# ljubobratovicrelja/tensor-truth

Hardware: AMD Instinct MI355X
Metric: queries/sec (embed+top-k+rerank) over 10M x 1024 corpus (higher is better)
Workload: dtype bf16

## Files before the change

tensor-truth_amd/csrc/scan.h:

```cpp
#pragma once
#include "common.h"

struct ScanParams {
    const uint16_t* corpus;
    const uint16_t* queries;
    int64_t row_lo, row_hi;
    int n_queries;
    int32_t idx_base;
    float* dense;
    int64_t dense_stride;
    const float* thr;
    int32_t* cnt;
    float* cand_scores;
    int32_t* cand_idx;
    int cap;
    uint2* priv;
    int32_t* priv_cnt;
    int64_t group_stride;
    int64_t phys_rows;
    int prof_id;
    const int32_t* row_table;
    const int32_t* row_cnt;
    const int32_t* gather_rows;
    const int32_t* row_range;
};

#define TT_SCAN_PRIV_SLOTS 16
#define TT_SCAN_WAVES_PER_BLOCK 8
#define TT_SCAN_MAX_SEGMENTS 64
#define TT_SCAN_MAX_PIECES 256

int tt_scan_launch(const ScanParams& p, int dim, int mode, int out, int blocks, hipStream_t stream);

struct SelectParams {
    const float* scores;
    const int32_t* idx;
    int64_t stride;
    const int32_t* cnt;
    int m_fixed;
    int cap;
    int32_t idx_base;
    int k;
    float* out_scores;
    int32_t* out_idx;
    int64_t out_stride;
    const uint2* priv;
    const int32_t* priv_cnt;
    int n_sub;
    float* thr_out;
    int32_t* cnt_out;
    int32_t* overflow_flag;
    int min_valid;
    int thr_relax;
    int32_t* zero_cnt;
    int n_real;
    int n_seg;
    int32_t seg_off[TT_SCAN_MAX_PIECES + 1];
    int32_t seg_add[TT_SCAN_MAX_PIECES];
};

int tt_select_launch(const SelectParams& p, int n_queries, hipStream_t stream);

int tt_lexical_score_lists(const int32_t* q_terms, const float* q_weights, const int32_t* q_start, const int32_t* q_nnz, int n_q,
                           const int32_t* d_terms, const float* d_weights, const int64_t* d_start, const int32_t* d_nnz,
                           const int32_t* cand, const int32_t* cand_cnt, int64_t stride, int grid_cand, float dead, float* out_lex,
                           hipStream_t stream);
bool tt_select_fused_outputs(int k);
```

tensor-truth_amd/csrc/scan.hip:

```cpp
#include "common.h"
#include "scan.h"

namespace {

constexpr int kThreads = 512;
constexpr int kWaves = kThreads / TT_WAVE;
constexpr int kBM = 64;
constexpr int kNG = kBM / 32;
constexpr int kScratchPerWave = 4096;
constexpr int kPrivSlots = TT_SCAN_PRIV_SLOTS;

template <int D>
struct Cfg {
    static constexpr int kRowBytes = D * 2;
    static constexpr int kQImageBytes = kBM * kRowBytes;
    static constexpr int NCH = D / 64;
    static constexpr int NKS = D / 16;
    static constexpr int P1 = (NCH % 4 == 0) ? 4 : ((NCH % 6 == 0) ? 6 : 2);
    static constexpr int P0 = (NKS % 16 == 0) ? 16 : 8;
};

__device__ __forceinline__ uint4 ldg16(const uint16_t* p) {
    return *reinterpret_cast<const uint4*>(p);
}

typedef __attribute__((ext_vector_type(4))) unsigned int u32x4;
template <bool NT>
__device__ __forceinline__ uint4 ldg16c(const uint16_t* p) {
    if constexpr (NT) {
        const u32x4 v = __builtin_nontemporal_load(reinterpret_cast<const u32x4*>(p));
        return make_uint4(v[0], v[1], v[2], v[3]);
    } else {
        return *reinterpret_cast<const uint4*>(p);
    }
}

template <int OUT>
__device__ __forceinline__ void scan_epilogue(const ScanParams& p, f32x16 (&acc)[2], const float (&thr)[2],
                                              const bool (&qvalid)[2], int q0, int ql, int half, int64_t grp,
                                              int (&pcnt)[2], uint2* const (&pbase)[2]) {
    const int64_t row0 = p.row_lo + grp * 32;
    const bool tail = row0 + 32 > p.row_hi;
#pragma unroll
    for (int g = 0; g < 2; ++g) {
        const int q = q0 + g * 32 + ql;
        if constexpr (OUT == 2) {
            float mx = acc[g][0];
#pragma unroll
            for (int r = 1; r < 16; ++r) mx = fmaxf(mx, acc[g][r]);
            mx = fmaxf(mx, __shfl_xor(mx, 32, 64));
            if (qvalid[g] && half == 0) p.dense[(size_t)q * p.dense_stride + (size_t)grp] = mx;
        } else if constexpr (OUT == 1) {
            if (qvalid[g]) {
                float* dst = p.dense + (size_t)q * p.dense_stride + (size_t)(row0 - p.row_lo);
#pragma unroll
                for (int j = 0; j < 4; ++j) {
                    float4 v = make_float4(acc[g][4 * j], acc[g][4 * j + 1], acc[g][4 * j + 2], acc[g][4 * j + 3]);
                    *reinterpret_cast<float4*>(dst + 8 * j + 4 * half) = v;
                }
            }
        } else {
            const float t = thr[g];
            float mx = acc[g][0];
#pragma unroll
            for (int r = 1; r < 16; ++r) mx = fmaxf(mx, acc[g][r]);
            if (__any(mx >= t)) {
#pragma unroll
                for (int r = 0; r < 16; ++r) {
                    const int64_t row = row0 + (r & 3) + 8 * (r >> 2) + 4 * half;
                    bool ok = acc[g][r] >= t;
                    if (tail) ok = ok && (row < p.row_hi);
                    if (ok) {
                        const uint2 e = make_uint2(__float_as_uint(acc[g][r]), (uint32_t)(p.idx_base + (int32_t)row));
                        if (pcnt[g] < kPrivSlots) {
                            pbase[g][pcnt[g]] = e;
                        } else {
                            const int pos = atomicAdd(p.cnt + q, 1);
                            if (pos < p.cap) {
                                p.cand_scores[(size_t)q * p.cap + pos] = acc[g][r];
                                p.cand_idx[(size_t)q * p.cap + pos] = (int32_t)e.y;
                            }
                        }
                        ++pcnt[g];
                    }
                }
            }
        }
#pragma unroll
        for (int r = 0; r < 16; ++r) acc[g][r] = 0.f;
    }
}

template <int D, int MODE, int OUT, int VAR, bool G = false>
__global__ __launch_bounds__(kThreads) void scan_kernel(ScanParams p) {
    using C = Cfg<D>;
    extern __shared__ __attribute__((aligned(16))) char smem[];
    char* q_img = smem;
    const int tid = threadIdx.x;
    const int lane = tid & 63;
    const int wave = __builtin_amdgcn_readfirstlane(tid >> 6);
    char* scratch = smem + C::kQImageBytes + wave * kScratchPerWave;

    const int q0 = blockIdx.y * kBM;

    {
        constexpr int kPiecesPerRow = D / 8;
        constexpr int kPieces = kBM * kPiecesPerRow;
        for (int t = tid; t < kPieces; t += kThreads) {
            const int q = t / kPiecesPerRow;
            const int c = t % kPiecesPerRow;
            uint4 v = make_uint4(0, 0, 0, 0);
            if (q0 + q < p.n_queries) v = ldg16(p.queries + (size_t)(q0 + q) * D + c * 8);
            *reinterpret_cast<uint4*>(q_img + q * C::kRowBytes + ((c ^ (q & 15)) << 4)) = v;
        }
    }
    __syncthreads();

    const int ql = lane & 31;
    const int half = lane >> 5;
    float thr[kNG];
    bool qvalid[kNG];
#pragma unroll
    for (int g = 0; g < kNG; ++g) {
        const int q = q0 + g * 32 + ql;
        qvalid[g] = q < p.n_queries;
        thr[g] = __builtin_inff();
        if (OUT == 0 && qvalid[g]) thr[g] = p.thr[q];
    }
    int qoff[kNG];
#pragma unroll
    for (int g = 0; g < kNG; ++g) qoff[g] = (g * 32 + ql) * C::kRowBytes;
    const int qswz = ql & 15;

    if constexpr (MODE == 0) {
        if (p.row_cnt) {
            const int64_t n = *p.row_cnt;
            p.row_hi = p.row_lo + (n < p.row_hi - p.row_lo ? n : p.row_hi - p.row_lo);
            if (p.row_hi <= p.row_lo) return;
        }
    }
    const int32_t* gtab = nullptr;
    if constexpr (G) {
        const int32_t b = p.row_range[0];
        const int64_t n = (int64_t)p.row_range[1] - b;
        const int64_t span = p.row_hi - p.row_lo;
        p.row_hi = p.row_lo + (n < 0 ? 0 : (n < span ? n : span));
        gtab = p.gather_rows + b;
    }
    const int64_t n_groups = (p.row_hi - p.row_lo + 31) / 32;
    const int64_t per_blk = n_groups / gridDim.x;
    const int64_t rem = n_groups % gridDim.x;
    const int64_t b = blockIdx.x;
    const int64_t g_lo = b * per_blk + (b < rem ? b : rem);
    const int64_t g_hi = g_lo + per_blk + (b < rem ? 1 : 0);

    const uint16_t* corpus = p.corpus;
    const int64_t gstride = (OUT == 2 && p.group_stride > 1) ? p.group_stride : 1;
    const int64_t last_row = (OUT == 2 && p.group_stride > 1) ? p.phys_rows - 1 : p.row_hi - 1;

    f32x16 acc[kNG];
#pragma unroll
    for (int g = 0; g < kNG; ++g)
#pragma unroll
        for (int r = 0; r < 16; ++r) acc[g][r] = 0.f;

    int64_t grp = g_lo + wave;
    const int n_sub = gridDim.x * kWaves * 2;
    const int sub = (blockIdx.x * kWaves + wave) * 2 + half;
    int pcnt[kNG];
    uint2* pbase[kNG];
#pragma unroll
    for (int g = 0; g < kNG; ++g) {
        pcnt[g] = 0;
        pbase[g] = nullptr;
        if (OUT == 0) pbase[g] = p.priv + ((size_t)(q0 + g * 32 + ql) * n_sub + sub) * kPrivSlots;
    }

    if constexpr (MODE == 1) {
        constexpr int P = C::P1;
        uint4 ring[P][4];
        const int lrow = lane >> 3;
        const int lpiece = lane & 7;
        int32_t grow[4] = {0, 0, 0, 0}, grow_n[4] = {0, 0, 0, 0};
        auto gload = [&](int32_t(&dst)[4], int64_t g) {
#pragma unroll
            for (int j = 0; j < 4; ++j) {
                int64_t row = p.row_lo + g * 32 + 8 * j + lrow;
                row = row < last_row ? row : last_row;
                dst[j] = gtab[row];
            }
        };
        auto issue = [&](uint4(&dst)[4], int64_t g, int c, const int32_t(&gr)[4]) {
#pragma unroll
            for (int j = 0; j < 4; ++j) {
                int64_t row;
                if constexpr (G) {
                    row = gr[j];
                } else {
                    row = p.row_lo + g * gstride * 32 + 8 * j + lrow;
                    row = row < last_row ? row : last_row;
                }
                dst[j] = ldg16c<(VAR & 1) == 0>(corpus + (size_t)row * D + c * 64 + lpiece * 8);
            }
        };
        int woff[4];
#pragma unroll
        for (int j = 0; j < 4; ++j) {
            const int row = 8 * j + lrow;
            woff[j] = row * 128 + ((lpiece ^ ((row >> 1) & 7)) << 4);
        }
        const int rbase = ql * 128;
        const int rswz = (ql >> 1) & 7;

        if (grp < g_hi) {
            if constexpr (G) gload(grow, grp);
#pragma unroll
            for (int c = 0; c < P; ++c) issue(ring[c], grp, c, grow);
        }
        while (grp < g_hi) {
            const int64_t nxt = grp + kWaves;
            const bool has_next = nxt < g_hi;
            if constexpr (G) {
                if (has_next) gload(grow_n, nxt);
            }
#pragma unroll
            for (int c = 0; c < C::NCH; ++c) {
                const int s = c % P;
                if constexpr ((VAR & 2) == 0) {
#pragma unroll
                    for (int j = 0; j < 4; ++j)
                        *reinterpret_cast<uint4*>(scratch + woff[j]) = ring[s][j];
                } else {
#pragma unroll
                    for (int j = 0; j < 4; ++j)
                        asm volatile("" ::"v"(ring[s][j].x), "v"(ring[s][j].y), "v"(ring[s][j].z), "v"(ring[s][j].w));
                }
                __builtin_amdgcn_sched_barrier(0);
                if (c + P < C::NCH) {
                    issue(ring[s], grp, c + P, grow);
                } else if (has_next) {
                    issue(ring[s], nxt, c + P - C::NCH, grow_n);
                }
                __builtin_amdgcn_sched_barrier(0);
                if constexpr ((VAR & 6) == 0)
#pragma unroll
                for (int ks = 0; ks < 4; ++ks) {
                    const int piece = 2 * ks + half;
                    const uint4 av = *reinterpret_cast<const uint4*>(scratch + rbase + ((piece ^ rswz) << 4));
                    const bf16x8 a = __builtin_bit_cast(bf16x8, av);
                    const int kc = c * 8 + piece;
#pragma unroll
                    for (int g = 0; g < kNG; ++g) {
                        if constexpr ((VAR & 16) != 0) {
                            acc[g] = __builtin_amdgcn_mfma_f32_32x32x16_bf16(a, a, acc[g], 0, 0, 0);
                        } else {
                            const uint4 bv = *reinterpret_cast<const uint4*>(q_img + qoff[g] + ((kc ^ qswz) << 4));
                            if constexpr ((VAR & 8) != 0) {
                                asm volatile("" ::"v"(bv.x), "v"(bv.y), "v"(bv.z), "v"(bv.w), "v"(av.x), "v"(av.w));
                            } else {
                                acc[g] = __builtin_amdgcn_mfma_f32_32x32x16_bf16(a, __builtin_bit_cast(bf16x8, bv), acc[g], 0, 0, 0);
                            }
                        }
                    }
                }
            }
            scan_epilogue<OUT>(p, acc, thr, qvalid, q0, ql, half, grp, pcnt, pbase);
            grp = nxt;
            if constexpr (G) {
#pragma unroll
                for (int j = 0; j < 4; ++j) grow[j] = grow_n[j];
            }
        }
    } else {
        constexpr int P = C::P0;
        uint4 ring[P];
        auto phys = [&](int64_t g) {
            int64_t row = p.row_lo + g * gstride * 32 + ql;
            const int64_t last = p.row_table ? p.row_hi - 1 : last_row;
            row = row < last ? row : last;
            return p.row_table ? (int64_t)p.row_table[row] : row;
        };
        int64_t row_cur = grp < g_hi ? phys(grp) : 0, row_nxt = 0;
        auto issue = [&](uint4& dst, int64_t row, int ks) {
            dst = ldg16c<(VAR & 1) == 0>(corpus + (size_t)row * D + ks * 16 + half * 8);
        };
        if (grp < g_hi) {
#pragma unroll
            for (int k = 0; k < P; ++k) issue(ring[k], row_cur, k);
        }
        while (grp < g_hi) {
            const int64_t nxt = grp + kWaves;
            const bool has_next = nxt < g_hi;
            if (has_next) row_nxt = phys(nxt);
#pragma unroll
            for (int ks = 0; ks < C::NKS; ++ks) {
                const int s = ks % P;
                const bf16x8 a = __builtin_bit_cast(bf16x8, ring[s]);
                const int kc = 2 * ks + half;
                bf16x8 bfr[kNG];
#pragma unroll
                for (int g = 0; g < kNG; ++g) {
                    const uint4 bv = *reinterpret_cast<const uint4*>(q_img + qoff[g] + ((kc ^ qswz) << 4));
                    bfr[g] = __builtin_bit_cast(bf16x8, bv);
                }
#pragma unroll
                for (int g = 0; g < kNG; ++g)
                    acc[g] = __builtin_amdgcn_mfma_f32_32x32x16_bf16(a, bfr[g], acc[g], 0, 0, 0);
                __builtin_amdgcn_sched_barrier(0);
                if (ks + P < C::NKS) {
                    issue(ring[s], row_cur, ks + P);
                } else if (has_next) {
                    issue(ring[s], row_nxt, ks + P - C::NKS);
                }
                __builtin_amdgcn_sched_barrier(0);
            }
            scan_epilogue<OUT>(p, acc, thr, qvalid, q0, ql, half, grp, pcnt, pbase);
            grp = nxt;
            row_cur = row_nxt;
        }
    }
    if constexpr (OUT == 0) {
#pragma unroll
        for (int g = 0; g < kNG; ++g)
            p.priv_cnt[(size_t)(q0 + g * 32 + ql) * n_sub + sub] = pcnt[g] < kPrivSlots ? pcnt[g] : kPrivSlots;
    }
}

}

template <int D, int MODE, int OUT, int VAR, bool G = false>
static int launch_one(const ScanParams& p, int blocks, int q_tiles, hipStream_t stream) {
    using C = Cfg<D>;
    const size_t lds = (size_t)C::kQImageBytes + (MODE == 1 ? (size_t)kWaves * kScratchPerWave : 0);
    auto kern = scan_kernel<D, MODE, OUT, VAR, G>;
    TT_SET_MAX_LDS(kern, lds);
    {
        TtProfScope prof(p.prof_id ? p.prof_id : (OUT == 0 ? TT_K_SCAN_FILTER : TT_K_SCAN_SAMPLE), stream);
        hipLaunchKernelGGL(kern, dim3(blocks, q_tiles), dim3(kThreads), lds, stream, p);
    }
    TT_CHECK_LAUNCH();
    return TT_OK;
}

template <int D>
static int launch_d(const ScanParams& p, int mode, int out, int blocks, int q_tiles, hipStream_t stream) {
    const int load_mode = mode & 15;
    const int var = mode >> 4;
    if (p.row_range) {
        switch (out) {
            case 0: return launch_one<D, 1, 0, 0, true>(p, blocks, q_tiles, stream);
            case 1: return launch_one<D, 1, 1, 0, true>(p, blocks, q_tiles, stream);
            default: return launch_one<D, 1, 2, 0, true>(p, blocks, q_tiles, stream);
        }
    }
    if constexpr (D == 1024) {
        if (out == 0 && load_mode == 1) {
            switch (var) {
                case 1: return launch_one<D, 1, 0, 1>(p, blocks, q_tiles, stream);
#if TT_DIAG
                case 2: return launch_one<D, 1, 0, 2>(p, blocks, q_tiles, stream);
                case 4: return launch_one<D, 1, 0, 4>(p, blocks, q_tiles, stream);
                case 8: return launch_one<D, 1, 0, 8>(p, blocks, q_tiles, stream);
#endif
                default: break;
            }
        }
    }
    if (load_mode == 1) {
        switch (out) {
            case 0: return launch_one<D, 1, 0, 0>(p, blocks, q_tiles, stream);
            case 1: return launch_one<D, 1, 1, 0>(p, blocks, q_tiles, stream);
            default: return launch_one<D, 1, 2, 0>(p, blocks, q_tiles, stream);
        }
    }
    switch (out) {
        case 0: return launch_one<D, 0, 0, 0>(p, blocks, q_tiles, stream);
        case 1: return launch_one<D, 0, 1, 0>(p, blocks, q_tiles, stream);
        default: return launch_one<D, 0, 2, 0>(p, blocks, q_tiles, stream);
    }
}

int tt_scan_launch(const ScanParams& p, int dim, int mode, int out, int blocks, hipStream_t stream) {
    const int q_tiles = (p.n_queries + kBM - 1) / kBM;
    if (p.row_hi <= p.row_lo || q_tiles == 0) return TT_OK;
    const int64_t n_groups = (p.row_hi - p.row_lo + 31) / 32;
    const int64_t max_blocks = out != 0 ? n_groups : (n_groups + kWaves - 1) / kWaves;
    if (blocks > max_blocks) blocks = (int)max_blocks;
    if (blocks < 1) blocks = 1;
    switch (dim) {
        case 128: return launch_d<128>(p, mode, out, blocks, q_tiles, stream);
        case 256: return launch_d<256>(p, mode, out, blocks, q_tiles, stream);
        case 384: return launch_d<384>(p, mode, out, blocks, q_tiles, stream);
        case 512: return launch_d<512>(p, mode, out, blocks, q_tiles, stream);
        case 640: return launch_d<640>(p, mode, out, blocks, q_tiles, stream);
        case 768: return launch_d<768>(p, mode, out, blocks, q_tiles, stream);
        case 896: return launch_d<896>(p, mode, out, blocks, q_tiles, stream);
        case 1024: return launch_d<1024>(p, mode, out, blocks, q_tiles, stream);
        default:
            tt_set_error("tt_scan: dim %d not in the compiled set {128,256,...,1024: multiples of 128}", dim);
            return TT_E_UNSUPPORTED;
    }
}
```

tensor-truth_amd/csrc/scan_api.hip:

```cpp
#include <limits.h>
#include <string.h>

#include "common.h"
#include "scan.h"
#include "encoder.h"
#include "shadow.h"

static thread_local char g_err[512] = "";

void tt_set_error(const char* fmt, ...) {
    va_list ap;
    va_start(ap, fmt);
    vsnprintf(g_err, sizeof(g_err), fmt, ap);
    va_end(ap);
}

int tt_cu_count_cached() {
    static thread_local int cached_dev = -1;
    static thread_local int cached_cus = 0;
    int dev = 0;
    if (hipGetDevice(&dev) != hipSuccess) return -1;
    if (dev != cached_dev) {
        int cus = 0;
        if (hipDeviceGetAttribute(&cus, hipDeviceAttributeMultiprocessorCount, dev) != hipSuccess) return -1;
        cached_dev = dev;
        cached_cus = cus;
    }
    return cached_cus;
}

namespace {

constexpr int kCap = 16384;
constexpr int64_t kSampleRows = 32768;

struct Plan {
    bool gemm;
    int q256;
    int cap;
    size_t off_q256;
    bool dense_only;
    int64_t n0;
    int64_t stride;
    int qpad;
    int main_blocks;
    int n_sub;
    size_t off_dense, off_cs, off_ci, off_cnt, off_thr, off_priv, off_pcnt, total;
};

int filter_blocks(int64_t rows, int cus) {
    const int64_t groups = (rows + 31) / 32;
    const int64_t mb = (groups + TT_SCAN_WAVES_PER_BLOCK - 1) / TT_SCAN_WAVES_PER_BLOCK;
    int64_t b = cus > 0 ? cus : 256;
    if (b > mb) b = mb;
    if (b < 1) b = 1;
    return (int)b;
}

bool scan_gemm_enabled() {
    static const bool on = TT_DIAG_ENV_INT("TT_SCAN_GEMM", 1) != 0;
    return on;
}

Plan make_plan(int64_t n_rows, int dim, int n_queries, int k, int cus, bool allow_gemm = true) {
    Plan pl{};
    pl.qpad = (n_queries + 63) / 64 * 64;
    pl.cap = kCap;
    int64_t n0 = kSampleRows;
    if (n0 < (int64_t)128 * k) n0 = (int64_t)128 * k;
    pl.gemm = allow_gemm && scan_gemm_enabled() && n_queries > 64 && dim % 128 == 0 && n_rows >= 262144 && n_rows >= (int64_t)2048 * k;
    if (pl.gemm) {
        static const int64_t n0_env = TT_DIAG_ENV_INT("TT_SCAN_GEMM_N0", 0);
        n0 = n0_env > 0 ? n0_env : 131072;
        if (n0_env <= 0)
            while (n0 > 32768 && n0 * 64 > n_rows) n0 /= 2;
        if (n0 < (int64_t)512 * k) n0 = (int64_t)512 * k;
        if (n0 > n_rows / 2) n0 = n_rows / 2 / 32 * 32;
        n0 = n0 / 256 * 256;
        pl.q256 = (n_queries + 255) / 256 * 256;
        pl.qpad = pl.q256;
        int64_t cap = 4 * (int64_t)k * n_rows / n0 + 4096;
        if (cap < kCap) cap = kCap;
        if (cap > (1 << 20)) cap = 1 << 20;
        pl.cap = (int)((cap + 63) / 64 * 64);
    }
    if (n_rows < (int64_t)128 * k || n_rows <= 8192) {
        pl.dense_only = true;
        pl.n0 = n_rows;
        pl.stride = (n_rows + 31) / 32 * 32;
    } else {
        pl.dense_only = false;
        pl.n0 = n0 < n_rows ? n0 : n_rows;
        pl.stride = ((pl.n0 + 31) / 32 + 31) / 32 * 32;
    }
    size_t off = 0;
    pl.off_dense = off; off += tt_align_up((size_t)pl.qpad * pl.stride * sizeof(float), 256);
    pl.off_cs = off;    off += tt_align_up((size_t)pl.qpad * pl.cap * sizeof(float), 256);
    pl.off_ci = off;    off += tt_align_up((size_t)pl.qpad * pl.cap * sizeof(int32_t), 256);
    pl.off_cnt = off;   off += tt_align_up((size_t)pl.qpad * sizeof(int32_t), 256);
    pl.off_thr = off;   off += tt_align_up((size_t)pl.qpad * sizeof(float), 256);
    if (pl.gemm) {
        pl.off_q256 = off; off += tt_align_up((size_t)pl.q256 * dim * sizeof(uint16_t), 256);
        pl.main_blocks = 1;
        pl.n_sub = TT_SCAN_WAVES_PER_BLOCK * 2;
        pl.off_priv = off; off += tt_align_up((size_t)pl.qpad * pl.n_sub * TT_SCAN_PRIV_SLOTS * sizeof(uint2), 256);
        pl.off_pcnt = off; off += tt_align_up((size_t)pl.qpad * pl.n_sub * sizeof(int32_t), 256);
    } else if (!pl.dense_only) {
        pl.main_blocks = filter_blocks(n_rows, cus);
        pl.n_sub = pl.main_blocks * TT_SCAN_WAVES_PER_BLOCK * 2;
        pl.off_priv = off; off += tt_align_up((size_t)pl.qpad * pl.n_sub * TT_SCAN_PRIV_SLOTS * sizeof(uint2), 256);
        pl.off_pcnt = off; off += tt_align_up((size_t)pl.qpad * pl.n_sub * sizeof(int32_t), 256);
    }
    pl.total = off;
    return pl;
}

int check_common(const void* corpus, int64_t n_rows, int dim, const void* queries, int n_queries, int k,
                 const float* out_scores, const int32_t* out_idx) {
    TT_CHECK_ARG(n_rows >= 0 && n_rows < (int64_t)INT32_MAX, "n_rows=%lld out of range", (long long)n_rows);
    TT_CHECK_ARG(n_queries >= 0, "n_queries=%d", n_queries);
    TT_CHECK_ARG(k >= 1 && k <= 1024, "k=%d outside [1,1024]", k);
    TT_CHECK_ARG(dim > 0 && dim % 128 == 0 && dim <= 1024, "dim=%d must be a multiple of 128 and <= 1024", dim);
    if (n_queries == 0) return TT_OK;
    TT_CHECK_ARG(out_scores && out_idx, "null output pointer");
    TT_CHECK_ARG(queries && ((uintptr_t)queries % 16) == 0, "queries must be non-null and 16-byte aligned");
    if (n_rows > 0) TT_CHECK_ARG(corpus && ((uintptr_t)corpus % 16) == 0, "corpus must be non-null and 16-byte aligned");
    return TT_OK;
}

__global__ void relax_thr_kernel(float* thr, int n) {
    const int i = blockIdx.x * blockDim.x + threadIdx.x;
    if (i < n) {
        const float t = thr[i];
        if (t - t == 0.f) thr[i] = t - (fabsf(t) * 1.220703125e-4f + 2e-6f);
    }
}

__global__ void fill_f32_kernel(float* s, float v, int n) {
    const int i = blockIdx.x * blockDim.x + threadIdx.x;
    if (i < n) s[i] = v;
}

__global__ void fill_pad_kernel(float* s, int32_t* ix, int64_t n) {
    const int64_t i = (int64_t)blockIdx.x * blockDim.x + threadIdx.x;
    if (i < n) {
        s[i] = -__builtin_inff();
        ix[i] = -1;
    }
}

int scan_mode_from_env() {
#if TT_DIAG
    const char* e = getenv("TT_SCAN_MODE");
    if (e && e[0]) return atoi(e);
#endif
    return 1;
}

struct ShadowLayout { size_t off_be, off_dn, total; };
ShadowLayout shadow_layout(int64_t cap_rows, int dim) {
    ShadowLayout l{};
    const size_t r16 = (size_t)(cap_rows + 15) / 16 * 16;
    size_t off = tt_align_up((size_t)cap_rows * dim, 256);
    l.off_be = off; off += tt_align_up(r16 * sizeof(float), 256);
    l.off_dn = off; off += tt_align_up(r16 * sizeof(float), 256);
    l.total = off;
    return l;
}
struct ShadowPlan {
    int64_t n0, stride;
    int blocks, n_waves, capw, cap;
    size_t off_sample, off_ss, off_si, off_thr, off_planes, off_qinfo, off_list, off_wcnt, off_table, off_tcnt, off_dense, total;
};
ShadowPlan shadow_plan(int64_t n_rows, int dim, int n_queries, int k, int cus) {
    ShadowPlan pl{};
    int64_t n0 = kSampleRows;
    if (n0 < (int64_t)128 * k) n0 = (int64_t)128 * k;
    if (n0 < n_rows / 32) n0 = n_rows / 32 / 32 * 32;
    pl.n0 = n0 < n_rows ? n0 : n_rows;
    pl.stride = ((pl.n0 + 31) / 32 + 31) / 32 * 32;
    pl.blocks = cus > 0 ? cus : 256;
    const int64_t groups = (n_rows + 15) / 16;
    if ((int64_t)pl.blocks * kShadowWavesPerBlock > groups) pl.blocks = (int)((groups + kShadowWavesPerBlock - 1) / kShadowWavesPerBlock);
    if (pl.blocks < 1) pl.blocks = 1;
    pl.n_waves = pl.blocks * kShadowWavesPerBlock;
    int64_t cap = n_rows / 16;
    if (cap < 65536) cap = 65536;
    if (cap > (1 << 20)) cap = 1 << 20;
    if (cap > (n_rows + 31) / 32 * 32) cap = (n_rows + 31) / 32 * 32;
    pl.cap = (int)((cap + 31) / 32 * 32);
    int64_t capw = 4 * (int64_t)pl.cap / pl.n_waves;
    if (capw < 64) capw = 64;
    pl.capw = (int)capw;
    const int qpad = 64;
    size_t off = 0;
    auto take = [&](size_t bytes) { size_t o = off; off += tt_align_up(bytes, 256); return o; };
    pl.off_sample = take((size_t)qpad * pl.stride * sizeof(float));
    pl.off_ss = take((size_t)qpad * k * sizeof(float));
    pl.off_si = take((size_t)qpad * k * sizeof(int32_t));
    pl.off_thr = take((size_t)qpad * sizeof(float));
    pl.off_planes = take((size_t)(dim / 128) * 4 * 1024);
    pl.off_qinfo = take(32 * sizeof(float));
    pl.off_list = take((size_t)n_queries * pl.n_waves * pl.capw * sizeof(int32_t));
    pl.off_wcnt = take((size_t)n_queries * pl.n_waves * sizeof(int32_t));
    pl.off_table = take((size_t)n_queries * pl.cap * sizeof(int32_t));
    pl.off_tcnt = take((size_t)qpad * sizeof(int32_t));
    pl.off_dense = take((size_t)pl.cap * sizeof(float));
    pl.total = off;
    return pl;
}
__global__ void add_idx_base_kernel(int32_t* idx, int n, int32_t base) {
    const int i = blockIdx.x * blockDim.x + threadIdx.x;
    if (i < n && idx[i] >= 0) idx[i] += base;
}

bool rows_dense(int64_t bound, int k) { return bound < (int64_t)128 * k || bound <= 8192; }
size_t rows_head_bytes(int n_queries) { return tt_align_up((size_t)((n_queries + 63) / 64 * 64) * sizeof(int32_t), 256); }
size_t rows_body_bytes(int64_t bound, int dim, int n_queries, int k, int cus) {
    if (bound <= 0) return 0;
    if (rows_dense(bound, k)) return tt_align_up((size_t)((n_queries + 63) / 64 * 64) * (size_t)((bound + 31) / 32 * 32) * sizeof(float), 256);
    return make_plan(bound, dim, n_queries, k, cus, false).total;
}
__global__ void rows_count_kernel(const int32_t* off, int s, int64_t bound, int32_t* cnt_q, int n, int32_t* flag) {
    const int i = blockIdx.x * blockDim.x + threadIdx.x;
    const int64_t c = (int64_t)off[s + 1] - off[s];
    if (i < n) cnt_q[i] = (int32_t)(c < bound ? c : bound);
    if (i == 0 && c > bound && flag) atomicOr(flag, 8);
}
__global__ void rows_map_kernel(int32_t* idx, int n_queries, int k, int64_t stride, const int32_t* rows, const int32_t* off, int s, int32_t add) {
    const int i = blockIdx.x * blockDim.x + threadIdx.x;
    if (i >= n_queries * k) return;
    int32_t* e = idx + (size_t)(i / k) * stride + (i % k);
    const int32_t pos = *e;
    if (pos >= 0) *e = rows[(int64_t)off[s] + pos] + add;
}
__global__ void fill_pad_strided_kernel(float* s, int32_t* ix, int n_queries, int width, int64_t stride) {
    const int i = blockIdx.x * blockDim.x + threadIdx.x;
    if (i < n_queries * width) {
        const size_t o = (size_t)(i / width) * stride + (i % width);
        s[o] = -__builtin_inff();
        ix[o] = -1;
    }
}
}

extern "C" {

int tt_version(void) { return 1; }
const char* tt_arch(void) { return "gfx950"; }
const char* tt_last_error(void) { return g_err; }
int tt_device_cu_count(void) { return tt_cu_count_cached(); }

size_t tt_scan_workspace_bytes(int64_t n_rows, int dim, int n_queries, int k) {
    if (n_rows < 0 || n_queries <= 0 || k < 1) return 0;
    int cus = tt_cu_count_cached();
    if (cus <= 0) cus = 256;
    return make_plan(n_rows, dim, n_queries, k, cus).total;
}

size_t tt_scan_exact_workspace_bytes(int64_t n_rows, int dim, int n_queries, int k) {
    (void)dim; (void)k;
    if (n_rows < 0 || n_queries <= 0) return 0;
    const int qpad = (n_queries + 63) / 64 * 64;
    const int64_t stride = (n_rows + 31) / 32 * 32;
    return tt_align_up((size_t)qpad * stride * sizeof(float), 256);
}

static int scan_dense_select(const void* corpus, int64_t n_rows, int dim, const void* queries, int n_queries,
                             int k, int32_t idx_base, float* out_scores, int32_t* out_idx, float* dense,
                             int64_t stride, hipStream_t st) {
    ScanParams sp{};
    sp.corpus = (const uint16_t*)corpus;
    sp.queries = (const uint16_t*)queries;
    sp.row_lo = 0;
    sp.row_hi = n_rows;
    sp.n_queries = n_queries;
    sp.idx_base = idx_base;
    sp.dense = dense;
    sp.dense_stride = stride;
    int rc = tt_scan_launch(sp, dim, scan_mode_from_env(), 1, tt_cu_count_cached(), st);
    if (rc) return rc;
    SelectParams se{};
    se.scores = dense;
    se.idx = nullptr;
    se.stride = stride;
    se.cnt = nullptr;
    se.m_fixed = (int)n_rows;
    se.cap = INT_MAX;
    se.idx_base = idx_base;
    se.k = k;
    se.out_scores = out_scores;
    se.out_idx = out_idx;
    se.out_stride = k;
    return tt_select_launch(se, n_queries, st);
}

int tt_scan_topk_exact(const void* corpus_bf16, int64_t n_rows, int dim, const void* queries_bf16,
                       int n_queries, int k, int32_t idx_base, float* out_scores, int32_t* out_idx,
                       void* workspace, size_t workspace_bytes, void* stream) {
    int rc = check_common(corpus_bf16, n_rows, dim, queries_bf16, n_queries, k, out_scores, out_idx);
    if (rc) return rc;
    if (n_queries == 0) return TT_OK;
    hipStream_t st = (hipStream_t)stream;
    if (n_rows == 0) {
        const int64_t n = (int64_t)n_queries * k;
        hipLaunchKernelGGL(fill_pad_kernel, dim3((unsigned)((n + 255) / 256)), dim3(256), 0, st, out_scores, out_idx, n);
        TT_CHECK_LAUNCH();
        return TT_OK;
    }
    const size_t need = tt_scan_exact_workspace_bytes(n_rows, dim, n_queries, k);
    if (!workspace || workspace_bytes < need) {
        tt_set_error("tt_scan_topk_exact: workspace %zu < required %zu bytes", workspace_bytes, need);
        return TT_E_WORKSPACE;
    }
    const int64_t stride = (n_rows + 31) / 32 * 32;
    return scan_dense_select(corpus_bf16, n_rows, dim, queries_bf16, n_queries, k, idx_base, out_scores, out_idx,
                             (float*)workspace, stride, st);
}

int tt_scan_topk(const void* corpus_bf16, int64_t n_rows, int dim, const void* queries_bf16, int n_queries,
                 int k, int32_t idx_base, float* out_scores, int32_t* out_idx, void* workspace,
                 size_t workspace_bytes, int32_t* status_flag, void* stream) {
    int rc = check_common(corpus_bf16, n_rows, dim, queries_bf16, n_queries, k, out_scores, out_idx);
    if (rc) return rc;
    if (n_queries == 0) return TT_OK;
    hipStream_t st = (hipStream_t)stream;
    if (status_flag) TT_CHECK_HIP(hipMemsetAsync(status_flag, 0, sizeof(int32_t), st));
    if (n_rows == 0) {
        const int64_t n = (int64_t)n_queries * k;
        hipLaunchKernelGGL(fill_pad_kernel, dim3((unsigned)((n + 255) / 256)), dim3(256), 0, st, out_scores, out_idx, n);
        TT_CHECK_LAUNCH();
        return TT_OK;
    }
    int cus_plan = tt_cu_count_cached();
    if (cus_plan <= 0) cus_plan = 256;
    const Plan pl = make_plan(n_rows, dim, n_queries, k, cus_plan);
    if (!workspace || workspace_bytes < pl.total) {
        tt_set_error("tt_scan_topk: workspace %zu < required %zu bytes", workspace_bytes, pl.total);
        return TT_E_WORKSPACE;
    }
    TT_CHECK_ARG(((uintptr_t)workspace % 256) == 0, "workspace must be 256-byte aligned");
    char* ws = (char*)workspace;
    float* dense = (float*)(ws + pl.off_dense);
    if (pl.dense_only) {
        return scan_dense_select(corpus_bf16, n_rows, dim, queries_bf16, n_queries, k, idx_base, out_scores,
                                 out_idx, dense, pl.stride, st);
    }
    float* cs = (float*)(ws + pl.off_cs);
    int32_t* ci = (int32_t*)(ws + pl.off_ci);
    int32_t* cnt = (int32_t*)(ws + pl.off_cnt);
    float* thr = (float*)(ws + pl.off_thr);
    const int mode = scan_mode_from_env();
    const int cus = tt_cu_count_cached();

    const uint16_t* q256 = (const uint16_t*)queries_bf16;
    if (pl.gemm && n_queries != pl.q256) {
        uint16_t* qpad256 = (uint16_t*)(ws + pl.off_q256);
        TT_CHECK_HIP(hipMemsetAsync(qpad256 + (size_t)n_queries * dim, 0, (size_t)(pl.q256 - n_queries) * dim * sizeof(uint16_t), st));
        TT_CHECK_HIP(hipMemcpyAsync(qpad256, queries_bf16, (size_t)n_queries * dim * sizeof(uint16_t), hipMemcpyDeviceToDevice, st));
        q256 = qpad256;
    }
    ScanParams sp{};
    sp.corpus = (const uint16_t*)corpus_bf16;
    sp.queries = (const uint16_t*)queries_bf16;
    sp.row_lo = 0;
    sp.row_hi = pl.n0;
    sp.n_queries = n_queries;
    sp.idx_base = idx_base;
    sp.dense = dense;
    sp.dense_stride = pl.stride;
    sp.group_stride = (n_rows / 32) / ((pl.n0 + 31) / 32);
    sp.phys_rows = n_rows;
    static const bool gemm_sample = TT_DIAG_ENV_INT("TT_SCAN_GEMM_SAMPLE", 1) != 0;
    if (pl.gemm && gemm_sample) {
        const int tiles = (int)(pl.n0 / 256);
        const int tile_stride = (int)((n_rows / 256) / tiles);
        for (int b = 0; b < pl.q256 / 256; ++b) {
            rc = tt_scan_gemm_sample_launch((const uint16_t*)corpus_bf16, tiles, tile_stride, dim, q256 + (size_t)b * 256 * dim, thr + b * 256,
                                            dense + (size_t)b * 256 * pl.stride, (int)pl.stride, st);
            if (rc) return rc;
        }
    } else {
        rc = tt_scan_launch(sp, dim, mode, 2, cus, st);
        if (rc) return rc;
    }

    SelectParams s1{};
    s1.scores = dense;
    s1.idx = nullptr;
    s1.stride = pl.stride;
    s1.cnt = nullptr;
    s1.m_fixed = (int)((pl.n0 + 31) / 32);
    s1.cap = INT_MAX;
    s1.idx_base = 0;
    s1.k = k;
    s1.out_scores = cs;
    s1.out_idx = ci;
    s1.out_stride = pl.cap;
    s1.thr_out = thr;
    s1.cnt_out = nullptr;
    const bool fused = tt_select_fused_outputs(k);
    if (fused) {
        s1.n_real = n_queries;
        s1.zero_cnt = cnt;
        s1.thr_relax = pl.gemm ? 1 : 0;
        rc = tt_select_launch(s1, pl.qpad, st);
        if (rc) return rc;
    } else {
        if (pl.gemm) {
            hipLaunchKernelGGL(fill_f32_kernel, dim3((pl.q256 + 255) / 256), dim3(256), 0, st, thr, __builtin_inff(), pl.q256);
            TT_CHECK_LAUNCH();
        }
        rc = tt_select_launch(s1, n_queries, st);
        if (rc) return rc;
    }
    if (pl.gemm && !fused) {
        hipLaunchKernelGGL(relax_thr_kernel, dim3((n_queries + 255) / 256), dim3(256), 0, st, thr, n_queries);
        TT_CHECK_LAUNCH();
    }
    if (!fused) TT_CHECK_HIP(hipMemsetAsync(cnt, 0, (size_t)pl.qpad * sizeof(int32_t), st));

    if (pl.gemm) {
        static const bool tail_pass = TT_DIAG_ENV_INT("TT_SCAN_GEMM_TAIL", 0) == 1;
        const int64_t rows256 = tail_pass ? n_rows / 256 * 256 : n_rows;
        for (int b = 0; b < pl.q256 / 256; ++b) {
            rc = tt_scan_gemm_launch((const uint16_t*)corpus_bf16, rows256, dim, q256 + (size_t)b * 256 * dim, thr + b * 256,
                                     cnt + b * 256, cs + (size_t)b * 256 * pl.cap, ci + (size_t)b * 256 * pl.cap, pl.cap, idx_base, st);
            if (rc) return rc;
        }
        SelectParams s2{};
        if (rows256 < n_rows) {
            ScanParams tp = sp;
            tp.group_stride = 0;
            tp.row_lo = rows256;
            tp.row_hi = n_rows;
            tp.dense = nullptr;
            tp.thr = thr;
            tp.cnt = cnt;
            tp.cand_scores = cs;
            tp.cand_idx = ci;
            tp.cap = pl.cap;
            tp.priv = (uint2*)(ws + pl.off_priv);
            tp.priv_cnt = (int32_t*)(ws + pl.off_pcnt);
            tp.prof_id = TT_K_SCAN_TAIL;
            rc = tt_scan_launch(tp, dim, mode, 0, 1, st);
            if (rc) return rc;
            s2.priv = tp.priv;
            s2.priv_cnt = tp.priv_cnt;
            s2.n_sub = pl.n_sub;
        }
        s2.scores = cs;
        s2.idx = ci;
        s2.stride = pl.cap;
        s2.cnt = cnt;
        s2.cap = pl.cap;
        s2.k = k;
        s2.out_scores = out_scores;
        s2.out_idx = out_idx;
        s2.out_stride = k;
        s2.overflow_flag = status_flag;
        s2.min_valid = (int)(n_rows < (int64_t)k ? n_rows : (int64_t)k);
        return tt_select_launch(s2, n_queries, st);
    }

    ScanParams mp = sp;
    mp.group_stride = 0;
    mp.row_lo = 0;
    mp.row_hi = n_rows;
    mp.dense = nullptr;
    mp.thr = thr;
    mp.cnt = cnt;
    mp.cand_scores = cs;
    mp.cand_idx = ci;
    mp.cap = pl.cap;
    mp.priv = (uint2*)(ws + pl.off_priv);
    mp.priv_cnt = (int32_t*)(ws + pl.off_pcnt);
    rc = tt_scan_launch(mp, dim, mode, 0, pl.main_blocks, st);
    if (rc) return rc;

    SelectParams s2{};
    s2.scores = cs;
    s2.idx = ci;
    s2.stride = pl.cap;
    s2.cnt = cnt;
    s2.m_fixed = 0;
    s2.cap = pl.cap;
    s2.k = k;
    s2.out_scores = out_scores;
    s2.out_idx = out_idx;
    s2.out_stride = k;
    s2.overflow_flag = status_flag;
    s2.priv = mp.priv;
    s2.priv_cnt = mp.priv_cnt;
    s2.n_sub = pl.n_sub;
    return tt_select_launch(s2, n_queries, st);
}

size_t tt_scan_shadow_bytes(int64_t cap_rows, int dim) {
    if (cap_rows <= 0 || dim <= 0 || dim % 128 || dim > 1024) return 0;
    return shadow_layout(cap_rows, dim).total;
}

int tt_scan_shadow_build(const void* corpus_bf16, int dim, int64_t row_lo, int64_t row_hi, void* shadow, int64_t cap_rows, void* stream) {
    TT_CHECK_ARG(dim > 0 && dim % 128 == 0 && dim <= 1024, "dim=%d must be a multiple of 128 and <= 1024", dim);
    TT_CHECK_ARG(row_lo >= 0 && row_lo <= row_hi && row_hi <= cap_rows, "rows [%lld, %lld) outside the shadow's capacity %lld", (long long)row_lo,
                 (long long)row_hi, (long long)cap_rows);
    if (row_hi == row_lo) return TT_OK;
    TT_CHECK_ARG(corpus_bf16 && shadow && ((uintptr_t)corpus_bf16 % 16) == 0 && ((uintptr_t)shadow % 256) == 0, "null or misaligned pointer");
    const ShadowLayout l = shadow_layout(cap_rows, dim);
    char* sb = (char*)shadow;
    return tt_shadow_build_launch((const uint16_t*)corpus_bf16 + (size_t)row_lo * dim, row_hi - row_lo, dim, (uint8_t*)sb + (size_t)row_lo * dim,
                                  (float*)(sb + l.off_be) + row_lo, (float*)(sb + l.off_dn) + row_lo, (hipStream_t)stream);
}

size_t tt_scan_shadow_workspace_bytes(int64_t n_rows, int dim, int n_queries, int k) {
    if (n_rows <= 0 || n_queries <= 0 || n_queries > 4 || k < 1 || dim <= 0 || dim % 128) return 0;
    int cus = tt_cu_count_cached();
    if (cus <= 0) cus = 256;
    return shadow_plan(n_rows, dim, n_queries, k, cus).total;
}

int tt_scan_topk_shadow(const void* corpus_bf16, const void* shadow, int64_t cap_rows, int64_t n_rows, int dim, const void* queries_bf16,
                        int n_queries, int k, int32_t idx_base, float* out_scores, int32_t* out_idx, void* workspace, size_t workspace_bytes,
                        int32_t* status_flag, void* stream) {
    int rc = check_common(corpus_bf16, n_rows, dim, queries_bf16, n_queries, k, out_scores, out_idx);
    if (rc) return rc;
    if (n_queries == 0) return TT_OK;
    TT_CHECK_ARG(n_queries <= 4, "n_queries=%d: the shadow prefilter serves lone callers (<= 4 queries per call)", n_queries);
    TT_CHECK_ARG(shadow && ((uintptr_t)shadow % 256) == 0 && n_rows <= cap_rows, "shadow missing, misaligned or smaller than n_rows");
    TT_CHECK_ARG(n_rows >= (int64_t)128 * k && n_rows > 8192, "n_rows=%lld: shards this small take tt_scan_topk's dense path", (long long)n_rows);
    hipStream_t st = (hipStream_t)stream;
    if (status_flag) TT_CHECK_HIP(hipMemsetAsync(status_flag, 0, sizeof(int32_t), st));
    int cus = tt_cu_count_cached();
    if (cus <= 0) cus = 256;
    const ShadowPlan pl = shadow_plan(n_rows, dim, n_queries, k, cus);
    if (!workspace || workspace_bytes < pl.total) {
        tt_set_error("tt_scan_topk_shadow: workspace %zu < required %zu bytes", workspace_bytes, pl.total);
        return TT_E_WORKSPACE;
    }
    TT_CHECK_ARG(((uintptr_t)workspace % 256) == 0, "workspace must be 256-byte aligned");
    char* ws = (char*)workspace;
    float* sample = (float*)(ws + pl.off_sample);
    float* thr = (float*)(ws + pl.off_thr);
    const int mode = scan_mode_from_env();
    ScanParams sp{};
    sp.corpus = (const uint16_t*)corpus_bf16;
    sp.queries = (const uint16_t*)queries_bf16;
    sp.row_lo = 0;
    sp.row_hi = pl.n0;
    sp.n_queries = n_queries;
    sp.dense = sample;
    sp.dense_stride = pl.stride;
    sp.group_stride = (n_rows / 32) / ((pl.n0 + 31) / 32);
    sp.phys_rows = n_rows;
    rc = tt_scan_launch(sp, dim, mode, 2, cus, st);
    if (rc) return rc;
    SelectParams s1{};
    s1.scores = sample;
    s1.stride = pl.stride;
    s1.m_fixed = (int)((pl.n0 + 31) / 32);
    s1.cap = INT_MAX;
    s1.k = k;
    s1.out_scores = (float*)(ws + pl.off_ss);
    s1.out_idx = (int32_t*)(ws + pl.off_si);
    s1.out_stride = k;
    s1.thr_out = thr;
    rc = tt_select_launch(s1, n_queries, st);
    if (rc) return rc;
    const ShadowLayout l = shadow_layout(cap_rows, dim);
    const char* sb = (const char*)shadow;
    uint16_t* planes = (uint16_t*)(ws + pl.off_planes);
    float* qinfo = (float*)(ws + pl.off_qinfo);
    int32_t* list = (int32_t*)(ws + pl.off_list);
    int32_t* wcnt = (int32_t*)(ws + pl.off_wcnt);
    int32_t* table = (int32_t*)(ws + pl.off_table);
    int32_t* tcnt = (int32_t*)(ws + pl.off_tcnt);
    rc = tt_shadow_query_launch((const uint16_t*)queries_bf16, n_queries, dim, planes, qinfo, st);
    if (rc) return rc;
    rc = tt_shadow_filter_launch((const uint8_t*)sb, (const float*)(sb + l.off_be), (const float*)(sb + l.off_dn), n_rows, dim, planes, qinfo, thr,
                                 n_queries, pl.blocks, list, wcnt, pl.capw, status_flag, st);
    if (rc) return rc;
    rc = tt_shadow_compact_launch(list, wcnt, pl.n_waves, pl.capw, n_queries, table, pl.cap, tcnt, status_flag, st);
    if (rc) return rc;
    float* dense = (float*)(ws + pl.off_dense);
    for (int q = 0; q < n_queries; ++q) {
        ScanParams rp{};
        rp.corpus = (const uint16_t*)corpus_bf16;
        rp.queries = (const uint16_t*)queries_bf16 + (size_t)q * dim;
        rp.row_lo = 0;
        rp.row_hi = pl.cap;
        rp.n_queries = 1;
        rp.dense = dense;
        rp.dense_stride = pl.cap;
        rp.row_table = table + (size_t)q * pl.cap;
        rp.row_cnt = tcnt + q;
        rp.prof_id = TT_K_SCAN_TAIL;
        rc = tt_scan_launch(rp, dim, 0, 1, cus, st);
        if (rc) return rc;
        SelectParams s2{};
        s2.scores = dense;
        s2.idx = table + (size_t)q * pl.cap;
        s2.stride = pl.cap;
        s2.cnt = tcnt + q;
        s2.cap = pl.cap;
        s2.k = k;
        s2.out_scores = out_scores + (size_t)q * k;
        s2.out_idx = out_idx + (size_t)q * k;
        s2.out_stride = k;
        s2.overflow_flag = status_flag;
        rc = tt_select_launch(s2, 1, st);
        if (rc) return rc;
    }
    if (idx_base != 0) {
        const int n = n_queries * k;
        hipLaunchKernelGGL(add_idx_base_kernel, dim3((n + 255) / 256), dim3(256), 0, st, out_idx, n, idx_base);
        TT_CHECK_LAUNCH();
    }
    return TT_OK;
}

size_t tt_scan_topk_rows_workspace_bytes(int64_t max_rows, int dim, int n_queries, int k) {
    if (max_rows < 0 || n_queries <= 0 || k < 1 || k > 1024) return 0;
    int cus = tt_cu_count_cached();
    if (cus <= 0) cus = 256;
    const int64_t dense_max = (int64_t)128 * k - 1 > 8192 ? (int64_t)128 * k - 1 : 8192;
    const size_t a = rows_body_bytes(max_rows, dim, n_queries, k, cus);
    const size_t b = rows_body_bytes(max_rows < dense_max ? max_rows : dense_max, dim, n_queries, k, cus);
    return rows_head_bytes(n_queries) + (a > b ? a : b);
}

int tt_scan_topk_rows(const void* corpus_bf16, int64_t n_rows, int dim, const void* queries_bf16, int n_queries, int k,
                      const int32_t* rows, const int32_t* list_offsets, int64_t max_rows, const int64_t* seg_offsets_host, int n_segments,
                      int32_t idx_base, float* out_scores, int32_t* out_idx, void* workspace, size_t workspace_bytes,
                      int32_t* status_flag, void* stream) {
    int rc = check_common(corpus_bf16, n_rows, dim, queries_bf16, n_queries, k, out_scores, out_idx);
    if (rc) return rc;
    TT_CHECK_ARG(n_segments >= 1 && n_segments <= TT_SCAN_MAX_SEGMENTS, "n_segments=%d outside [1,%d]", n_segments, TT_SCAN_MAX_SEGMENTS);
    TT_CHECK_ARG(max_rows >= 0, "max_rows=%lld", (long long)max_rows);
    if (seg_offsets_host) {
        TT_CHECK_ARG(seg_offsets_host[0] >= 0 && seg_offsets_host[n_segments] <= n_rows, "segment offsets outside [0, n_rows]");
        for (int s = 0; s < n_segments; ++s)
            TT_CHECK_ARG(seg_offsets_host[s] <= seg_offsets_host[s + 1], "segment offsets must be non-decreasing (segment %d)", s);
    } else {
        TT_CHECK_ARG(n_segments == 1, "n_segments=%d without segment offsets", n_segments);
    }
    if (n_queries == 0) return TT_OK;
    TT_CHECK_ARG(list_offsets && (rows || max_rows == 0), "null row list");
    hipStream_t st = (hipStream_t)stream;
    if (status_flag) TT_CHECK_HIP(hipMemsetAsync(status_flag, 0, sizeof(int32_t), st));
    int cus = tt_cu_count_cached();
    if (cus <= 0) cus = 256;
    const size_t need = tt_scan_topk_rows_workspace_bytes(max_rows, dim, n_queries, k);
    if (!workspace || workspace_bytes < need) {
        tt_set_error("tt_scan_topk_rows: workspace %zu < required %zu bytes", workspace_bytes, need);
        return TT_E_WORKSPACE;
    }
    TT_CHECK_ARG(((uintptr_t)workspace % 256) == 0, "workspace must be 256-byte aligned");
    const int qpad = (n_queries + 63) / 64 * 64;
    int32_t* cnt_q = (int32_t*)workspace;
    char* ws = (char*)workspace + rows_head_bytes(n_queries);
    const int64_t ostride = (int64_t)n_segments * k;
    const int mode = 1;
    {
        const int n = n_queries * n_segments * k;
        hipLaunchKernelGGL(fill_pad_strided_kernel, dim3((n + 255) / 256), dim3(256), 0, st, out_scores, out_idx, 1, n, (int64_t)n);
        TT_CHECK_LAUNCH();
    }
    for (int s = 0; s < n_segments; ++s) {
        const int64_t seg_rows = seg_offsets_host ? seg_offsets_host[s + 1] - seg_offsets_host[s] : n_rows;
        const int64_t bound = max_rows < seg_rows ? max_rows : seg_rows;
        if (bound <= 0) continue;
        float* os = out_scores + (size_t)s * k;
        int32_t* oi = out_idx + (size_t)s * k;
        hipLaunchKernelGGL(rows_count_kernel, dim3((qpad + 255) / 256), dim3(256), 0, st, list_offsets, s, bound, cnt_q, qpad, status_flag);
        TT_CHECK_LAUNCH();
        ScanParams sp{};
        sp.corpus = (const uint16_t*)corpus_bf16;
        sp.queries = (const uint16_t*)queries_bf16;
        sp.row_lo = 0;
        sp.n_queries = n_queries;
        sp.gather_rows = rows;
        sp.row_range = list_offsets + s;
        if (rows_dense(bound, k)) {
            const int64_t stride = (bound + 31) / 32 * 32;
            sp.row_hi = bound;
            sp.dense = (float*)ws;
            sp.dense_stride = stride;
            rc = tt_scan_launch(sp, dim, mode, 1, cus, st);
            if (rc) return rc;
            SelectParams se{};
            se.scores = (float*)ws;
            se.stride = stride;
            se.cnt = cnt_q;
            se.cap = INT_MAX;
            se.k = k;
            se.out_scores = os;
            se.out_idx = oi;
            se.out_stride = ostride;
            rc = tt_select_launch(se, n_queries, st);
            if (rc) return rc;
        } else {
            const Plan pl = make_plan(bound, dim, n_queries, k, cus, false);
            float* dense = (float*)(ws + pl.off_dense);
            float* cs = (float*)(ws + pl.off_cs);
            int32_t* ci = (int32_t*)(ws + pl.off_ci);
            int32_t* cnt = (int32_t*)(ws + pl.off_cnt);
            float* thr = (float*)(ws + pl.off_thr);
            {
                const int n = pl.qpad * (int)pl.stride;
                hipLaunchKernelGGL(fill_f32_kernel, dim3((n + 255) / 256), dim3(256), 0, st, dense, -__builtin_inff(), n);
                TT_CHECK_LAUNCH();
            }
            sp.row_hi = pl.n0;
            sp.dense = dense;
            sp.dense_stride = pl.stride;
            rc = tt_scan_launch(sp, dim, mode, 2, cus, st);
            if (rc) return rc;
            SelectParams s1{};
            s1.scores = dense;
            s1.stride = pl.stride;
            s1.m_fixed = (int)((pl.n0 + 31) / 32);
            s1.cap = INT_MAX;
            s1.k = k;
            s1.out_scores = cs;
            s1.out_idx = ci;
            s1.out_stride = pl.cap;
            s1.thr_out = thr;
            if (tt_select_fused_outputs(k)) {
                s1.n_real = n_queries;
                s1.zero_cnt = cnt;
                rc = tt_select_launch(s1, pl.qpad, st);
                if (rc) return rc;
            } else {
                rc = tt_select_launch(s1, n_queries, st);
                if (rc) return rc;
                TT_CHECK_HIP(hipMemsetAsync(cnt, 0, (size_t)pl.qpad * sizeof(int32_t), st));
            }
            ScanParams mp = sp;
            mp.row_hi = bound;
            mp.dense = nullptr;
            mp.thr = thr;
            mp.cnt = cnt;
            mp.cand_scores = cs;
            mp.cand_idx = ci;
            mp.cap = pl.cap;
            mp.priv = (uint2*)(ws + pl.off_priv);
            mp.priv_cnt = (int32_t*)(ws + pl.off_pcnt);
            rc = tt_scan_launch(mp, dim, mode, 0, pl.main_blocks, st);
            if (rc) return rc;
            SelectParams s2{};
            s2.scores = cs;
            s2.idx = ci;
            s2.stride = pl.cap;
            s2.cnt = cnt;
            s2.cap = pl.cap;
            s2.k = k;
            s2.out_scores = os;
            s2.out_idx = oi;
            s2.out_stride = ostride;
            s2.overflow_flag = status_flag;
            s2.priv = mp.priv;
            s2.priv_cnt = mp.priv_cnt;
            s2.n_sub = pl.n_sub;
            rc = tt_select_launch(s2, n_queries, st);
            if (rc) return rc;
        }
        const int n = n_queries * k;
        const int32_t add = seg_offsets_host ? (int32_t)(-seg_offsets_host[s]) : idx_base;
        hipLaunchKernelGGL(rows_map_kernel, dim3((n + 255) / 256), dim3(256), 0, st, oi, n_queries, k, ostride, rows, list_offsets, s, add);
        TT_CHECK_LAUNCH();
    }
    return TT_OK;
}

constexpr int64_t kPieceRows = 65536;

static size_t seg_dense_bytes(int64_t rows, int n_queries) {
    return tt_align_up((size_t)n_queries * (size_t)((rows + 31) / 32 * 32) * sizeof(float), 256);
}

size_t tt_scan_segmented_workspace_bytes(int64_t n_rows, int dim, int n_queries, int k) {
    (void)dim;
    if (n_rows < 0 || n_queries <= 0 || k < 1) return 0;
    return seg_dense_bytes(n_rows, n_queries) + 2 * tt_align_up((size_t)n_queries * TT_SCAN_MAX_PIECES * k * 4, 256);
}

int tt_scan_topk_segmented(const void* corpus_bf16, int64_t n_rows, int dim, const void* queries_bf16,
                           int n_queries, int k, const int64_t* seg_offsets, int n_segments, float* out_scores,
                           int32_t* out_idx, void* workspace, size_t workspace_bytes, void* stream) {
    int rc = check_common(corpus_bf16, n_rows, dim, queries_bf16, n_queries, k, out_scores, out_idx);
    if (rc) return rc;
    TT_CHECK_ARG(n_segments >= 1 && n_segments <= TT_SCAN_MAX_SEGMENTS, "n_segments=%d outside [1,%d]", n_segments,
                 TT_SCAN_MAX_SEGMENTS);
    TT_CHECK_ARG(seg_offsets != nullptr, "null seg_offsets");
    TT_CHECK_ARG(seg_offsets[0] >= 0 && seg_offsets[n_segments] <= n_rows, "segment offsets outside [0, n_rows]");
    for (int s = 0; s < n_segments; ++s)
        TT_CHECK_ARG(seg_offsets[s] <= seg_offsets[s + 1], "segment offsets must be non-decreasing (segment %d)", s);
    if (n_queries == 0) return TT_OK;
    hipStream_t st = (hipStream_t)stream;
    const int64_t lo = seg_offsets[0], rows = seg_offsets[n_segments] - lo;
    if (rows == 0) {
        const int64_t n = (int64_t)n_queries * n_segments * k;
        hipLaunchKernelGGL(fill_pad_kernel, dim3((unsigned)((n + 255) / 256)), dim3(256), 0, st, out_scores, out_idx, n);
        TT_CHECK_LAUNCH();
        return TT_OK;
    }
    const size_t need = tt_scan_segmented_workspace_bytes(rows, dim, n_queries, k);
    if (!workspace || workspace_bytes < need) {
        tt_set_error("tt_scan_topk_segmented: workspace %zu < required %zu bytes", workspace_bytes, need);
        return TT_E_WORKSPACE;
    }
    TT_CHECK_ARG(((uintptr_t)workspace % 16) == 0, "workspace must be 16-byte aligned");
    const int64_t stride = (rows + 31) / 32 * 32;
    ScanParams sp{};
    sp.corpus = (const uint16_t*)corpus_bf16 + (size_t)lo * dim;
    sp.queries = (const uint16_t*)queries_bf16;
    sp.row_lo = 0;
    sp.row_hi = rows;
    sp.n_queries = n_queries;
    sp.dense = (float*)workspace;
    sp.dense_stride = stride;
    rc = tt_scan_launch(sp, dim, scan_mode_from_env(), 1, tt_cu_count_cached(), st);
    if (rc) return rc;

    int64_t piece_rows = kPieceRows;
    const int64_t spare = TT_SCAN_MAX_PIECES - n_segments;
    if ((rows + piece_rows - 1) / piece_rows > spare) piece_rows = (rows + spare - 1) / spare;
    SelectParams se{};
    int first_piece[TT_SCAN_MAX_SEGMENTS + 1];
    int n_pieces = 0;
    for (int s = 0; s < n_segments; ++s) {
        first_piece[s] = n_pieces;
        const int64_t b = seg_offsets[s] - lo, e = seg_offsets[s + 1] - lo;
        int64_t pos = b;
        do {
            const int64_t end = (e - pos > piece_rows) ? pos + piece_rows : e;
            se.seg_off[n_pieces] = (int32_t)pos;
            se.seg_add[n_pieces] = (int32_t)(pos - b);
            ++n_pieces;
            pos = end;
        } while (pos < e);
    }
    first_piece[n_segments] = n_pieces;
    se.seg_off[n_pieces] = (int32_t)rows;
    se.scores = sp.dense;
    se.stride = stride;
    se.cap = INT_MAX;
    se.k = k;
    se.out_stride = k;
    se.n_seg = n_pieces;
    if (n_pieces == n_segments) {
        se.out_scores = out_scores;
        se.out_idx = out_idx;
        return tt_select_launch(se, n_queries, st);
    }
    char* tmp = (char*)workspace + seg_dense_bytes(rows, n_queries);
    float* part_s = (float*)tmp;
    int32_t* part_i = (int32_t*)(tmp + tt_align_up((size_t)n_queries * TT_SCAN_MAX_PIECES * k * 4, 256));
    se.out_scores = part_s;
    se.out_idx = part_i;
    rc = tt_select_launch(se, n_queries, st);
    if (rc) return rc;
    SelectParams sm{};
    sm.scores = part_s;
    sm.idx = part_i;
    sm.stride = (int64_t)n_pieces * k;
    sm.cap = INT_MAX;
    sm.k = k;
    sm.out_scores = out_scores;
    sm.out_idx = out_idx;
    sm.out_stride = k;
    sm.n_seg = n_segments;
    for (int s = 0; s <= n_segments; ++s) sm.seg_off[s] = first_piece[s] * k;
    return tt_select_launch(sm, n_queries, st);
}

int tt_topk_merge(const float* in_scores, const int32_t* in_idx, int n_queries, int n_candidates, int k_out,
                  float* out_scores, int32_t* out_idx, void* stream) {
    TT_CHECK_ARG(n_queries >= 0 && n_candidates >= 0, "negative size");
    TT_CHECK_ARG(k_out >= 1 && k_out <= 1024, "k_out=%d outside [1,1024]", k_out);
    if (n_queries == 0) return TT_OK;
    TT_CHECK_ARG(in_scores && in_idx && out_scores && out_idx, "null pointer");
    SelectParams se{};
    se.scores = in_scores;
    se.idx = in_idx;
    se.stride = n_candidates;
    se.cnt = nullptr;
    se.m_fixed = n_candidates;
    se.cap = INT_MAX;
    se.k = k_out;
    se.out_scores = out_scores;
    se.out_idx = out_idx;
    se.out_stride = k_out;
    return tt_select_launch(se, n_queries, (hipStream_t)stream);
}

}
```

tensor-truth_amd/csrc/shadow.h:

```cpp
#pragma once
#include "common.h"

constexpr int kShadowWavesPerBlock = 8;
int tt_shadow_build_launch(const uint16_t* corpus, int64_t n_rows, int dim, uint8_t* shadow, float* be, float* dn, hipStream_t st);
int tt_shadow_query_launch(const uint16_t* queries, int n_queries, int dim, uint16_t* frags, float* qinfo, hipStream_t st);
int tt_shadow_filter_launch(const uint8_t* shadow, const float* be, const float* dn, int64_t n_rows, int dim, const uint16_t* frags,
                            const float* qinfo, const float* thr, int n_queries, int blocks, int32_t* list, int32_t* wave_cnt, int capw,
                            int32_t* status_flag, hipStream_t st);
int tt_shadow_compact_launch(const int32_t* list, const int32_t* wave_cnt, int n_waves, int capw, int n_queries, int32_t* table, int cap,
                             int32_t* table_cnt, int32_t* status_flag, hipStream_t st);
```

tensor-truth_amd/csrc/shadow.hip:

```cpp
#include "common.h"
#include "scan.h"
#include "shadow.h"

namespace {

typedef int v8i __attribute__((ext_vector_type(8)));
typedef float f4 __attribute__((ext_vector_type(4)));
constexpr float kShadowScale = 256.0f;
constexpr int kSWaves = 8, kSThreads = 64 * kSWaves;

__device__ __forceinline__ float bf16_to_f32(uint16_t b) { return __uint_as_float((uint32_t)b << 16); }
__device__ __forceinline__ uint32_t to_e4m3(float x) {
    const float c = x != x ? x : __builtin_amdgcn_fmed3f(x, -448.0f, 448.0f);
    return (uint32_t)__builtin_amdgcn_cvt_pk_fp8_f32(c, c, 0, false) & 0xFFu;
}
__device__ __forceinline__ float from_e4m3(uint32_t byte) { return __builtin_amdgcn_cvt_f32_fp8((int)byte, 0); }

__global__ __launch_bounds__(256) void shadow_build_kernel(const uint16_t* corpus, int64_t n_rows, int dim, uint8_t* shadow, float* be, float* dn) {
    const int64_t row = (int64_t)blockIdx.x * 4 + (threadIdx.x >> 6);
    const int lane = threadIdx.x & 63;
    if (row >= n_rows) return;
    float se = 0.f, sd = 0.f;
    for (int c = lane * 8; c < dim; c += 512) {
        const uint4 v = *reinterpret_cast<const uint4*>(corpus + (size_t)row * dim + c);
        const uint32_t w[4] = {v.x, v.y, v.z, v.w};
        uint32_t out[2] = {0u, 0u};
#pragma unroll
        for (int i = 0; i < 8; ++i) {
            const float x = bf16_to_f32((uint16_t)(i & 1 ? w[i >> 1] >> 16 : w[i >> 1] & 0xFFFFu));
            const uint32_t b = to_e4m3(x * kShadowScale);
            const float d = from_e4m3(b) * (1.0f / kShadowScale);
            const float e = x - d;
            se = fmaf(e, e, se);
            sd = fmaf(d, d, sd);
            out[i >> 2] |= b << (8 * (i & 3));
        }
        *reinterpret_cast<uint2*>(shadow + (size_t)row * dim + c) = make_uint2(out[0], out[1]);
    }
    se = wave_sum(se);
    sd = wave_sum(sd);
    if (lane == 0) {
        be[row] = sqrtf(se) * 1.0005f + 1e-9f;
        dn[row] = sqrtf(sd) * 1.0005f + 1e-9f;
    }
}

__global__ __launch_bounds__(64) void shadow_query_kernel(const uint16_t* queries, int n_queries, int dim, uint16_t* frags, float* qinfo) {
    const int q = blockIdx.x, lane = threadIdx.x;
    float sq = 0.f;
    for (int c = lane; c < dim; c += 64) {
        uint16_t v = 0;
        if (q < n_queries) v = queries[(size_t)q * dim + c];
        const float x = bf16_to_f32(v);
        sq = fmaf(x, x, sq);
        const int kt = c >> 7, g4 = (c & 127) >> 5, f = (c & 31) >> 3, e = c & 7;
        frags[((size_t)(kt * 4 + f) * 64 + (g4 * 16 + q)) * 8 + e] = v;
    }
    sq = wave_sum(sq);
    if (lane == 0) qinfo[q] = sqrtf(sq) * 1.0005f + 1e-9f;
}

struct ShadowParams {
    const uint8_t* shadow;
    const float* be;
    const float* dn;
    const uint16_t* frags;
    const float* qinfo;
    const float* thr;
    int64_t n_rows;
    int n_queries;
    int32_t* list;
    int32_t* wave_cnt;
    int capw;
    int32_t* status_flag;
};

template <bool HI>
__device__ __forceinline__ uint32_t e4m3x2_to_bf16x2(uint32_t w) {
    const auto f = __builtin_amdgcn_cvt_pk_f32_fp8((int)w, HI);
    return __builtin_amdgcn_perm(__float_as_uint(f[1]), __float_as_uint(f[0]), 0x07060302u);
}

template <int D>
__global__ __launch_bounds__(kSThreads, 2) void shadow_filter_kernel(ShadowParams p) {
    constexpr int NKT = D / 128;
    extern __shared__ __attribute__((aligned(16))) char smem[];
    uint4* qf = reinterpret_cast<uint4*>(smem);
    int* lcnt = reinterpret_cast<int*>(smem + NKT * 4 * 1024);
    const int tid = threadIdx.x, lane = tid & 63;
    const int wave = __builtin_amdgcn_readfirstlane(tid >> 6);
    char* scratch = smem + NKT * 4 * 1024 + kSWaves * 16 * sizeof(int) + wave * 2048;
    for (int i = tid; i < NKT * 4 * 64; i += kSThreads) qf[i] = reinterpret_cast<const uint4*>(p.frags)[i];
    if (tid < kSWaves * 16) lcnt[tid] = 0;
    __syncthreads();

    const int j = lane & 15, g4 = lane >> 4;
    const bool qok = j < p.n_queries;
    const float thr = qok ? p.thr[j] : __builtin_inff();
    const float qn = p.qinfo[j];
    const int n_waves = gridDim.x * kSWaves;
    const int wg = blockIdx.x * kSWaves + wave;
    const int64_t n_groups = (p.n_rows + 15) / 16;
    typedef unsigned int u32x4 __attribute__((ext_vector_type(4)));
    const int lrow = lane >> 3, lpiece = lane & 7;
    const int woff0 = lrow * 128 + ((lpiece ^ ((lrow >> 1) & 7)) << 4);
    const int woff1 = (8 + lrow) * 128 + ((lpiece ^ (((8 + lrow) >> 1) & 7)) << 4);
    const int roff0 = j * 128 + (((2 * g4) ^ ((j >> 1) & 7)) << 4);
    const int roff1 = j * 128 + (((2 * g4 + 1) ^ ((j >> 1) & 7)) << 4);

    auto load_group = [&](u32x4 (&a)[NKT][2], int64_t grp) {
        int64_t r0 = grp * 16 + lrow, r1 = r0 + 8;
        r0 = r0 < p.n_rows ? r0 : p.n_rows - 1;
        r1 = r1 < p.n_rows ? r1 : p.n_rows - 1;
        const u32x4* s0 = reinterpret_cast<const u32x4*>(p.shadow + (size_t)r0 * D + lpiece * 16);
        const u32x4* s1 = reinterpret_cast<const u32x4*>(p.shadow + (size_t)r1 * D + lpiece * 16);
#pragma unroll
        for (int kt = 0; kt < NKT; ++kt) {
            a[kt][0] = __builtin_nontemporal_load(s0 + kt * 8);
            a[kt][1] = __builtin_nontemporal_load(s1 + kt * 8);
        }
    };
    auto process = [&](const u32x4 (&a)[NKT][2], int64_t grp) {
        f32x4 acc = f32x4{0.f, 0.f, 0.f, 0.f};
#pragma unroll
        for (int kt = 0; kt < NKT; ++kt) {
            *reinterpret_cast<u32x4*>(scratch + woff0) = a[kt][0];
            *reinterpret_cast<u32x4*>(scratch + woff1) = a[kt][1];
            const u32x4 x0 = *reinterpret_cast<const u32x4*>(scratch + roff0);
            const u32x4 x1 = *reinterpret_cast<const u32x4*>(scratch + roff1);
#pragma unroll
            for (int f = 0; f < 4; ++f) {
                const uint32_t w0 = (f < 2 ? x0 : x1)[(f & 1) * 2], w1 = (f < 2 ? x0 : x1)[(f & 1) * 2 + 1];
                const uint4 av = make_uint4(e4m3x2_to_bf16x2<false>(w0), e4m3x2_to_bf16x2<true>(w0), e4m3x2_to_bf16x2<false>(w1),
                                            e4m3x2_to_bf16x2<true>(w1));
                const uint4 bv = qf[(kt * 4 + f) * 64 + lane];
                acc = TT_MFMA_16x16x32(__builtin_bit_cast(ex8, av), __builtin_bit_cast(ex8, bv), acc);
            }
        }
        const int64_t r0 = grp * 16 + g4 * 4;
        const float4 be4 = *reinterpret_cast<const float4*>(p.be + r0);
        const float4 dn4 = *reinterpret_cast<const float4*>(p.dn + r0);
        const float bes[4] = {be4.x, be4.y, be4.z, be4.w};
        const float dns[4] = {dn4.x, dn4.y, dn4.z, dn4.w};
        constexpr float kGamma2 = 2.0f * (float)(D + 8) * 1.1920928955078125e-7f;
#pragma unroll
        for (int r = 0; r < 4; ++r) {
            const float ub = acc[r] * (1.0f / kShadowScale) + qn * bes[r] + (kGamma2 * qn * (dns[r] + bes[r]) + 1e-30f);
            if (qok && ub >= thr && r0 + r < p.n_rows) {
                const int pos = atomicAdd(&lcnt[wave * 16 + j], 1);
                if (pos < p.capw) p.list[((size_t)j * n_waves + wg) * p.capw + pos] = (int32_t)(r0 + r);
            }
        }
    };

    u32x4 a0[NKT][2], a1[NKT][2];
    int64_t grp = wg;
    if (grp < n_groups) load_group(a0, grp);
    while (grp < n_groups) {
        const int64_t g1 = grp + n_waves, g2 = g1 + n_waves;
        if (g1 < n_groups) load_group(a1, g1);
        process(a0, grp);
        if (g1 >= n_groups) break;
        if (g2 < n_groups) load_group(a0, g2);
        process(a1, g1);
        grp = g2;
    }
    asm volatile("s_waitcnt lgkmcnt(0)" ::: "memory");
    __builtin_amdgcn_wave_barrier();
    if (lane < p.n_queries) {
        const int c = reinterpret_cast<volatile int*>(lcnt)[wave * 16 + lane];
        p.wave_cnt[(size_t)lane * n_waves + wg] = c < p.capw ? c : p.capw;
        if (c > p.capw && p.status_flag) atomicOr(p.status_flag, 2);
    }
}

__global__ __launch_bounds__(1024) void shadow_compact_kernel(const int32_t* list, const int32_t* wave_cnt, int n_waves, int capw, int32_t* table,
                                                              int cap, int32_t* table_cnt, int32_t* status_flag) {
    __shared__ int wsum[16];
    __shared__ int total;
    const int q = blockIdx.x, tid = threadIdx.x, lane = tid & 63, wv = tid >> 6;
    const int32_t* cnts = wave_cnt + (size_t)q * n_waves;
    const int per = (n_waves + 1023) / 1024;
    int mine = 0;
    for (int i = 0; i < per; ++i) {
        const int w = tid * per + i;
        if (w < n_waves) mine += cnts[w];
    }
    int inc = mine;
#pragma unroll
    for (int o = 1; o < 64; o <<= 1) {
        const int v = __shfl_up(inc, o, 64);
        if (lane >= o) inc += v;
    }
    if (lane == 63) wsum[wv] = inc;
    __syncthreads();
    int base = 0;
    for (int i = 0; i < wv; ++i) base += wsum[i];
    if (tid == 1023) total = base + inc;
    int off = base + inc - mine;
    for (int i = 0; i < per; ++i) {
        const int w = tid * per + i;
        if (w >= n_waves) break;
        const int c = cnts[w];
        const int32_t* src = list + ((size_t)q * n_waves + w) * capw;
        for (int e = 0; e < c; ++e)
            if (off + e < cap) table[(size_t)q * cap + off + e] = src[e];
        off += c;
    }
    __syncthreads();
    if (tid == 0) {
        table_cnt[q] = total < cap ? total : cap;
        if (total > cap && status_flag) atomicOr(status_flag, 4);
    }
}

}

int tt_shadow_build_launch(const uint16_t* corpus, int64_t n_rows, int dim, uint8_t* shadow, float* be, float* dn, hipStream_t st) {
    if (n_rows <= 0) return TT_OK;
    hipLaunchKernelGGL(shadow_build_kernel, dim3((unsigned)((n_rows + 3) / 4)), dim3(256), 0, st, corpus, n_rows, dim, shadow, be, dn);
    TT_CHECK_LAUNCH();
    return TT_OK;
}

int tt_shadow_query_launch(const uint16_t* queries, int n_queries, int dim, uint16_t* frags, float* qinfo, hipStream_t st) {
    hipLaunchKernelGGL(shadow_query_kernel, dim3(16), dim3(64), 0, st, queries, n_queries, dim, frags, qinfo);
    TT_CHECK_LAUNCH();
    return TT_OK;
}

template <int D>
static int launch_filter(const ShadowParams& p, int blocks, hipStream_t st) {
    constexpr size_t lds = (D / 128) * 4 * 1024 + kSWaves * 16 * sizeof(int) + kSWaves * 2048;
    TT_SET_MAX_LDS(shadow_filter_kernel<D>, lds);
    {
        TtProfScope prof(TT_K_SCAN_FILTER, st);
        hipLaunchKernelGGL(shadow_filter_kernel<D>, dim3(blocks), dim3(kSThreads), lds, st, p);
    }
    TT_CHECK_LAUNCH();
    return TT_OK;
}

int tt_shadow_filter_launch(const uint8_t* shadow, const float* be, const float* dn, int64_t n_rows, int dim, const uint16_t* frags,
                            const float* qinfo, const float* thr, int n_queries, int blocks, int32_t* list, int32_t* wave_cnt, int capw,
                            int32_t* status_flag, hipStream_t st) {
    ShadowParams p{};
    p.shadow = shadow; p.be = be; p.dn = dn; p.frags = frags; p.qinfo = qinfo; p.thr = thr; p.n_rows = n_rows; p.n_queries = n_queries;
    p.list = list; p.wave_cnt = wave_cnt; p.capw = capw; p.status_flag = status_flag;
    switch (dim) {
        case 128: return launch_filter<128>(p, blocks, st);
        case 256: return launch_filter<256>(p, blocks, st);
        case 384: return launch_filter<384>(p, blocks, st);
        case 512: return launch_filter<512>(p, blocks, st);
        case 640: return launch_filter<640>(p, blocks, st);
        case 768: return launch_filter<768>(p, blocks, st);
        case 896: return launch_filter<896>(p, blocks, st);
        case 1024: return launch_filter<1024>(p, blocks, st);
        default:
            tt_set_error("shadow scan: dim %d not in the compiled set {128, 256, ..., 1024}", dim);
            return TT_E_UNSUPPORTED;
    }
}

int tt_shadow_compact_launch(const int32_t* list, const int32_t* wave_cnt, int n_waves, int capw, int n_queries, int32_t* table, int cap,
                             int32_t* table_cnt, int32_t* status_flag, hipStream_t st) {
    TtProfScope prof(TT_K_SELECT, st);
    hipLaunchKernelGGL(shadow_compact_kernel, dim3(n_queries), dim3(1024), 0, st, list, wave_cnt, n_waves, capw, table, cap, table_cnt, status_flag);
    TT_CHECK_LAUNCH();
    return TT_OK;
}
```

tensor-truth_amd/scan.py:

```python
from __future__ import annotations

import threading
from typing import Optional, Tuple

import torch

from . import _lib


def _require_cuda(t: torch.Tensor, name: str) -> None:
    if not t.is_cuda:
        raise RuntimeError(
            f"{name} must live on a HIP device (got {t.device}); tensor_truth_amd has no CPU path"
        )


class _Workspace(threading.local):

    def __init__(self):
        self.bufs = {}

    def get(self, device: torch.device, nbytes: int) -> torch.Tensor:
        key = (device.type, device.index)
        buf = self.bufs.get(key)
        if buf is None or buf.numel() < nbytes:
            buf = torch.empty(max(nbytes, 1), dtype=torch.uint8, device=device)
            self.bufs[key] = buf
        return buf


_ws = _Workspace()


def _stream_ptr(device: torch.device) -> int:
    return torch.cuda.current_stream(device).cuda_stream


class ScanShadow:

    MIN_ROWS = 1 << 20
    MAX_QUERIES = 4

    def __init__(self, corpus: torch.Tensor, cap_rows: Optional[int] = None):
        _require_cuda(corpus, "corpus")
        if corpus.dtype != torch.bfloat16 or corpus.dim() != 2 or not corpus.is_contiguous():
            raise TypeError("the shadow mirrors a contiguous [N, D] torch.bfloat16 matrix")
        self.dim = int(corpus.shape[1])
        self.cap_rows = int(cap_rows if cap_rows is not None else corpus.shape[0])
        lib = _lib.load_library()
        nbytes = lib.tt_scan_shadow_bytes(self.cap_rows, self.dim)
        if nbytes == 0:
            raise ValueError(f"no shadow for {self.cap_rows} rows x {self.dim}")
        self._raw = torch.empty(nbytes + 256, dtype=torch.uint8, device=corpus.device)
        self.ptr = (self._raw.data_ptr() + 255) // 256 * 256
        self.rows = 0
        self.base_ptr = corpus.data_ptr()
        self.ready = torch.cuda.Event()
        self.extend(corpus, int(corpus.shape[0]))

    def extend(self, corpus: torch.Tensor, n_rows: int) -> None:
        if n_rows > self.cap_rows or corpus.shape[1] != self.dim:
            raise ValueError("the shadow's capacity / width does not fit this matrix")
        if n_rows <= self.rows:
            return
        lib = _lib.load_library()
        with torch.cuda.device(corpus.device):
            rc = lib.tt_scan_shadow_build(corpus.data_ptr(), self.dim, self.rows, n_rows, self.ptr, self.cap_rows, _stream_ptr(corpus.device))
            _lib.check(rc, "tt_scan_shadow_build")
            self.ready.record(torch.cuda.current_stream(corpus.device))
        self.rows = n_rows

    def rebuild(self, corpus: torch.Tensor, n_rows: int) -> None:
        self.rows = 0
        self.extend(corpus, n_rows)

    def serves(self, n_rows: int, n_queries: int, k: int) -> bool:
        return (self.rows >= n_rows >= max(self.MIN_ROWS, 128 * k) and 0 < n_queries <= self.MAX_QUERIES)


def scan_topk(
    corpus: torch.Tensor,
    queries: torch.Tensor,
    k: int,
    idx_base: int = 0,
    exact_dense: bool = False,
    check_overflow: bool = True,
    return_flag: bool = False,
    _packed: Optional[torch.Tensor] = None,
    shadow: Optional[ScanShadow] = None,
):
    lib = _lib.load_library()
    _require_cuda(corpus, "corpus")
    _require_cuda(queries, "queries")
    if corpus.dtype != torch.bfloat16 or queries.dtype != torch.bfloat16:
        raise TypeError("corpus and queries must be torch.bfloat16")
    if corpus.dim() != 2 or queries.dim() != 2 or corpus.shape[1] != queries.shape[1]:
        raise ValueError(f"shape mismatch: corpus {tuple(corpus.shape)} queries {tuple(queries.shape)}")
    if corpus.device != queries.device:
        raise ValueError("corpus and queries must be on the same device")
    if not corpus.is_contiguous() or not queries.is_contiguous():
        raise ValueError("corpus and queries must be contiguous row-major")
    n, d = corpus.shape
    q = queries.shape[0]
    dev = corpus.device
    if _packed is not None:
        out_s = _packed[: q * k].view(torch.float32).view(q, k)
        out_i = _packed[q * k: 2 * q * k].view(q, k)
    else:
        out_s = torch.empty((q, k), dtype=torch.float32, device=dev)
        out_i = torch.empty((q, k), dtype=torch.int32, device=dev)
    if q == 0:
        return out_s, out_i
    with torch.cuda.device(dev):
        st = _stream_ptr(dev)
        if exact_dense:
            need = lib.tt_scan_exact_workspace_bytes(n, d, q, k)
            ws = _ws.get(dev, need)
            rc = lib.tt_scan_topk_exact(corpus.data_ptr(), n, d, queries.data_ptr(), q, k, idx_base,
                                        out_s.data_ptr(), out_i.data_ptr(), ws.data_ptr(), ws.numel(), st)
            _lib.check(rc, "tt_scan_topk_exact")
            return out_s, out_i
        use_shadow = shadow is not None and shadow.dim == d and shadow.serves(n, q, k)
        need = lib.tt_scan_shadow_workspace_bytes(n, d, q, k) if use_shadow else lib.tt_scan_workspace_bytes(n, d, q, k)
        ws = _ws.get(dev, need + 256)
        base = (ws.data_ptr() + 255) // 256 * 256
        if _packed is not None:
            flag = _packed[2 * q * k:]
            flag.zero_()
        else:
            flag = torch.zeros(1, dtype=torch.int32, device=dev)
        if use_shadow:
            torch.cuda.current_stream(dev).wait_event(shadow.ready)
            rc = lib.tt_scan_topk_shadow(corpus.data_ptr(), shadow.ptr, shadow.cap_rows, n, d, queries.data_ptr(), q, k, idx_base,
                                         out_s.data_ptr(), out_i.data_ptr(), base, ws.numel() - (base - ws.data_ptr()),
                                         flag.data_ptr(), st)
            _lib.check(rc, "tt_scan_topk_shadow")
        else:
            rc = lib.tt_scan_topk(corpus.data_ptr(), n, d, queries.data_ptr(), q, k, idx_base,
                                  out_s.data_ptr(), out_i.data_ptr(), base, ws.numel() - (base - ws.data_ptr()),
                                  flag.data_ptr(), st)
            _lib.check(rc, "tt_scan_topk")
        if _packed is not None:
            return out_s, out_i
        if return_flag:
            return out_s, out_i, int(flag.item())
        if check_overflow and int(flag.item()) != 0:
            return scan_topk(corpus, queries, k, idx_base, exact_dense=True)
    return out_s, out_i


def scan_topk_host(corpus: torch.Tensor, queries: torch.Tensor, k: int, idx_base: int = 0, shadow: Optional[ScanShadow] = None):
    q = queries.shape[0]
    if q == 0:
        return torch.empty((0, k), dtype=torch.float32), torch.empty((0, k), dtype=torch.int32)
    packed = torch.empty(2 * q * k + 1, dtype=torch.int32, device=corpus.device)
    scan_topk(corpus, queries, k, idx_base, _packed=packed, shadow=shadow)
    host = packed.cpu()
    if int(host[-1]) != 0:
        s, i = scan_topk(corpus, queries, k, idx_base, exact_dense=True)
        return s.cpu(), i.cpu()
    return host[: q * k].view(torch.float32).view(q, k), host[q * k: 2 * q * k].view(q, k)


def scan_topk_segmented(corpus: torch.Tensor, queries: torch.Tensor, k: int, seg_offsets) -> Tuple[torch.Tensor, torch.Tensor]:
    import ctypes
    lib = _lib.load_library()
    _require_cuda(corpus, "corpus")
    _require_cuda(queries, "queries")
    if corpus.dtype != torch.bfloat16 or queries.dtype != torch.bfloat16:
        raise TypeError("corpus and queries must be torch.bfloat16")
    if corpus.dim() != 2 or queries.dim() != 2 or corpus.shape[1] != queries.shape[1]:
        raise ValueError(f"shape mismatch: corpus {tuple(corpus.shape)} queries {tuple(queries.shape)}")
    if corpus.device != queries.device:
        raise ValueError("corpus and queries must be on the same device")
    if not corpus.is_contiguous() or not queries.is_contiguous():
        raise ValueError("corpus and queries must be contiguous row-major")
    offs = [int(o) for o in seg_offsets]
    n_seg = len(offs) - 1
    if n_seg < 1:
        raise ValueError("seg_offsets needs at least two entries")
    n, d = corpus.shape
    q = queries.shape[0]
    dev = corpus.device
    out_s = torch.empty((q, n_seg, k), dtype=torch.float32, device=dev)
    out_i = torch.empty((q, n_seg, k), dtype=torch.int32, device=dev)
    if q == 0:
        return out_s, out_i
    c_offs = (ctypes.c_int64 * (n_seg + 1))(*offs)
    with torch.cuda.device(dev):
        need = lib.tt_scan_segmented_workspace_bytes(max(offs[-1] - offs[0], 0), d, q, k)
        ws = _ws.get(dev, need + 256)
        base = (ws.data_ptr() + 255) // 256 * 256
        rc = lib.tt_scan_topk_segmented(corpus.data_ptr(), n, d, queries.data_ptr(), q, k, c_offs, n_seg,
                                        out_s.data_ptr(), out_i.data_ptr(), base,
                                        ws.numel() - (base - ws.data_ptr()), _stream_ptr(dev))
        _lib.check(rc, "tt_scan_topk_segmented")
    return out_s, out_i


def filter_rows(compiled, n_rows: int, device, seg_offsets=None) -> Tuple[torch.Tensor, torch.Tensor]:
    import ctypes
    lib = _lib.load_library()
    offs = [0, int(n_rows)] if seg_offsets is None else [int(o) for o in seg_offsets]
    n_seg = len(offs) - 1
    span = offs[-1] - offs[0]
    rows = torch.empty(max(span, 1), dtype=torch.int32, device=device)
    list_off = torch.empty(n_seg + 1, dtype=torch.int32, device=device)
    n_cl = len(compiled.columns)
    c_codes = (ctypes.c_void_p * n_cl)(*[c.data_ptr() for c in compiled.columns])
    c_bits = (ctypes.c_void_p * n_cl)(*[b.data_ptr() for b in compiled.bitsets])
    c_ncodes = (ctypes.c_int32 * n_cl)(*compiled.n_codes)
    c_offs = (ctypes.c_int64 * (n_seg + 1))(*offs) if seg_offsets is not None else None
    with torch.cuda.device(device):
        need = lib.tt_filter_rows_workspace_bytes(span)
        ws = _filter_ws.get(device, need + 256)
        base = (ws.data_ptr() + 255) // 256 * 256
        rc = lib.tt_filter_rows(n_cl, c_codes, c_bits, c_ncodes, 1 if compiled.any else 0, int(n_rows), c_offs, n_seg,
                                rows.data_ptr(), list_off.data_ptr(), base, ws.numel() - (base - ws.data_ptr()), _stream_ptr(device))
        _lib.check(rc, "tt_filter_rows")
    return rows, list_off


_filter_ws = _Workspace()


def scan_topk_rows(corpus: torch.Tensor, queries: torch.Tensor, k: int, rows: torch.Tensor, list_offsets: torch.Tensor,
                   max_rows: int, seg_offsets=None, idx_base: int = 0, check_overflow: bool = True, return_flag: bool = False,
                   _packed: Optional[torch.Tensor] = None):
    import ctypes
    lib = _lib.load_library()
    _require_cuda(corpus, "corpus")
    _require_cuda(queries, "queries")
    if corpus.dtype != torch.bfloat16 or queries.dtype != torch.bfloat16:
        raise TypeError("corpus and queries must be torch.bfloat16")
    if corpus.dim() != 2 or queries.dim() != 2 or corpus.shape[1] != queries.shape[1]:
        raise ValueError(f"shape mismatch: corpus {tuple(corpus.shape)} queries {tuple(queries.shape)}")
    if not corpus.is_contiguous() or not queries.is_contiguous():
        raise ValueError("corpus and queries must be contiguous row-major")
    n, d = corpus.shape
    q = queries.shape[0]
    dev = corpus.device
    n_seg = 1 if seg_offsets is None else len(seg_offsets) - 1
    shape = (q, k) if seg_offsets is None else (q, n_seg, k)
    if _packed is not None:
        out_s = _packed[: q * n_seg * k].view(torch.float32).view(shape)
        out_i = _packed[q * n_seg * k: 2 * q * n_seg * k].view(shape)
    else:
        out_s = torch.empty(shape, dtype=torch.float32, device=dev)
        out_i = torch.empty(shape, dtype=torch.int32, device=dev)
    if q == 0:
        return out_s, out_i
    c_offs = (ctypes.c_int64 * (n_seg + 1))(*[int(o) for o in seg_offsets]) if seg_offsets is not None else None
    with torch.cuda.device(dev):
        st = _stream_ptr(dev)
        need = lib.tt_scan_topk_rows_workspace_bytes(int(max_rows), d, q, k)
        ws = _ws.get(dev, need + 256)
        base = (ws.data_ptr() + 255) // 256 * 256
        if _packed is not None:
            flag = _packed[2 * q * n_seg * k:]
            flag.zero_()
        else:
            flag = torch.zeros(1, dtype=torch.int32, device=dev)
        rc = lib.tt_scan_topk_rows(corpus.data_ptr(), n, d, queries.data_ptr(), q, k, rows.data_ptr(), list_offsets.data_ptr(),
                                   int(max_rows), c_offs, n_seg, idx_base, out_s.data_ptr(), out_i.data_ptr(), base,
                                   ws.numel() - (base - ws.data_ptr()), flag.data_ptr(), st)
        _lib.check(rc, "tt_scan_topk_rows")
        if _packed is not None:
            return out_s, out_i
        if return_flag:
            return out_s, out_i, int(flag.item())
        if check_overflow and int(flag.item()) != 0:
            return scan_topk_rows_exact(corpus, queries, k, rows, list_offsets, seg_offsets, idx_base)
    return out_s, out_i


def scan_topk_rows_exact(corpus, queries, k, rows, list_offsets, seg_offsets=None, idx_base: int = 0):
    offs = list_offsets.cpu().tolist()
    n_seg = len(offs) - 1
    q = queries.shape[0]
    s_out = torch.full((q, n_seg, k), float("-inf"), dtype=torch.float32, device=corpus.device)
    i_out = torch.full((q, n_seg, k), -1, dtype=torch.int32, device=corpus.device)
    for s in range(n_seg):
        sub = rows[offs[s]:offs[s + 1]].long()
        if sub.numel() == 0:
            continue
        es, ei = scan_topk(corpus.index_select(0, sub).contiguous(), queries, k, exact_dense=True)
        add = idx_base if seg_offsets is None else -int(seg_offsets[s])
        mapped = torch.where(ei >= 0, sub[ei.clamp_min(0).long()].to(torch.int32) + add, ei)
        s_out[:, s], i_out[:, s] = es, mapped
    if seg_offsets is None:
        return s_out[:, 0].contiguous(), i_out[:, 0].contiguous()
    return s_out, i_out


def scan_topk_rows_host(corpus, queries, k, rows, list_offsets, max_rows: int, seg_offsets=None, idx_base: int = 0):
    q = queries.shape[0]
    n_seg = 1 if seg_offsets is None else len(seg_offsets) - 1
    shape = (q, k) if seg_offsets is None else (q, n_seg, k)
    if q == 0:
        return torch.empty(shape, dtype=torch.float32), torch.empty(shape, dtype=torch.int32)
    m = q * n_seg * k
    packed = torch.empty(2 * m + 1, dtype=torch.int32, device=corpus.device)
    scan_topk_rows(corpus, queries, k, rows, list_offsets, max_rows, seg_offsets, idx_base, _packed=packed)
    host = packed.cpu()
    if int(host[-1]) != 0:
        s, i = scan_topk_rows_exact(corpus, queries, k, rows, list_offsets, seg_offsets, idx_base)
        return s.cpu(), i.cpu()
    return host[:m].view(torch.float32).view(shape), host[m: 2 * m].view(shape)


def topk_merge(scores: torch.Tensor, idx: torch.Tensor, k: int) -> Tuple[torch.Tensor, torch.Tensor]:
    lib = _lib.load_library()
    _require_cuda(scores, "scores")
    _require_cuda(idx, "idx")
    if scores.dtype != torch.float32 or idx.dtype != torch.int32:
        raise TypeError("scores must be float32 and idx int32")
    if scores.shape != idx.shape or scores.dim() != 2:
        raise ValueError("scores/idx must both be [Q, M]")
    scores = scores.contiguous()
    idx = idx.contiguous()
    q, m = scores.shape
    dev = scores.device
    out_s = torch.empty((q, k), dtype=torch.float32, device=dev)
    out_i = torch.empty((q, k), dtype=torch.int32, device=dev)
    if q == 0:
        return out_s, out_i
    with torch.cuda.device(dev):
        rc = lib.tt_topk_merge(scores.data_ptr(), idx.data_ptr(), q, m, k, out_s.data_ptr(), out_i.data_ptr(),
                               _stream_ptr(dev))
        _lib.check(rc, "tt_topk_merge")
    return out_s, out_i


def similarity_from_cosine(cos: torch.Tensor) -> torch.Tensor:
    return torch.exp(-(2.0 - 2.0 * cos))
```

tensor-truth_amd/sharded_index.py:

```python
from __future__ import annotations

import math
import os
import threading
from typing import Callable, Dict, List, Optional, Sequence, Tuple

import torch
import torch.distributed as dist

from . import _lib
from . import sharded as _sh
from .schema import NodeWithScore, TextNode
from .vector_index import (HipVectorIndex, HipVectorRetriever, _read_persisted, _node_from_dict)


def _world(group) -> Tuple[int, int]:
    if dist.is_available() and dist.is_initialized():
        return dist.get_world_size(group), dist.get_rank(group)
    return 1, 0


class ShardRoundError(RuntimeError):
    """A rank's local scan failed inside a collective round.  The failing rank still takes part in the round's all-gather
    (with a poisoned partial list), so EVERY rank raises this for the round's queries and nobody is left waiting in a collective."""


_POISON = -2


class ShardedHipVectorIndex:
    def __init__(self, dim: int, local_rows: torch.Tensor, row_lo: int, n_total: int, leaf_ids: Sequence[Optional[str]],
                 docstore: Dict[str, TextNode], embed_model=None, score_mode: str = "chroma", group=None,
                 logical_shards: int = 1, queries: str = "replicated", ragged_queries: bool = True,
                 scan_fn: Optional[Callable] = None, merge_fn: Optional[Callable] = None):
        if queries not in ("replicated", "partitioned"):
            raise ValueError("queries must be 'replicated' or 'partitioned'")
        if local_rows.dtype != torch.bfloat16 or local_rows.dim() != 2 or local_rows.shape[1] != dim:
            raise ValueError("local_rows must be a [n_local, dim] bfloat16 matrix")
        if leaf_ids is not None and len(leaf_ids) != n_total:
            raise ValueError(f"leaf_ids has {len(leaf_ids)} entries for {n_total} global rows")
        if scan_fn is None and not local_rows.is_cuda:
            raise RuntimeError("ShardedHipVectorIndex needs its shard on a HIP device; tensor_truth_amd has no CPU path")
        self.dim, self.device = dim, local_rows.device
        self.row_lo, self.n_total = int(row_lo), int(n_total)
        self.leaf_ids = leaf_ids if leaf_ids is None or not isinstance(leaf_ids, (list, tuple)) else list(leaf_ids)
        self.docstore = docstore
        self.embed_model = embed_model
        self.score_mode = score_mode
        self.group = group
        self.queries = queries
        self.ragged_queries = ragged_queries
        if scan_fn is None or merge_fn is None:
            from . import scan as _scan

            scan_fn = scan_fn or self._scan_shard
            merge_fn = merge_fn or _scan.topk_merge
        self._scan, self._merge = scan_fn, merge_fn
        self.fp8_shadow = os.environ.get("TT_SCAN_SHADOW", "1") != "0"
        self._shadows: Dict[int, object] = {}
        self._shadow_lock = threading.Lock()
        self._collective_lock = threading.Lock()
        self._tick_fronts = 0
        self._written = None
        if local_rows.is_cuda:
            self._written = torch.cuda.Event()
            self._written.record(torch.cuda.current_stream(local_rows.device))
        n_local = local_rows.shape[0]
        pieces = max(1, min(int(logical_shards), max(n_local, 1)))
        self._shards: List[Tuple[torch.Tensor, int]] = []
        for p in range(pieces):
            lo, hi = _sh.shard_bounds(n_local, pieces, p)
            self._shards.append((local_rows[lo:hi], self.row_lo + lo))

    @classmethod
    def from_index(cls, index: HipVectorIndex, group=None, **kw) -> "ShardedHipVectorIndex":
        world, rank = _world(group)
        index._compact()
        mat, leaf_ids = index.snapshot()
        lo, hi = _sh.shard_bounds(mat.shape[0], world, rank)
        return cls(index.dim, mat[lo:hi].contiguous(), lo, mat.shape[0], leaf_ids, index.docstore,
                   embed_model=kw.pop("embed_model", index.embed_model), score_mode=kw.pop("score_mode", index.score_mode),
                   group=group, **kw)

    @classmethod
    def from_local(cls, dim: int, local_rows: torch.Tensor, local_leaf_ids: Sequence[str], local_docstore: Dict[str, TextNode],
                   group=None, **kw) -> "ShardedHipVectorIndex":
        world, rank = _world(group)
        local_leaf_ids = list(local_leaf_ids)
        if local_rows.shape[0] != len(local_leaf_ids):
            raise ValueError(f"{local_rows.shape[0]} local rows but {len(local_leaf_ids)} local leaf ids")
        if world == 1:
            return cls(dim, local_rows, 0, len(local_leaf_ids), local_leaf_ids, dict(local_docstore), group=group, **kw)
        from .vector_index import _node_to_dict

        mine = (local_leaf_ids, {nid: _node_to_dict(nd) for nid, nd in local_docstore.items()})
        parts: List = [None] * world
        dist.all_gather_object(parts, mine, group=group)
        counts = [len(p[0]) for p in parts]
        leaf_ids: List[Optional[str]] = []
        docstore: Dict[str, TextNode] = {}
        for r, (ids, nodes) in enumerate(parts):
            leaf_ids.extend(ids)
            if r == rank:
                docstore.update(local_docstore)
            else:
                for nid, d in nodes.items():
                    docstore.setdefault(nid, _node_from_dict(nid, d))
        if len(set(i for i in leaf_ids if i is not None)) != sum(1 for i in leaf_ids if i is not None):
            raise ValueError("the ranks' leaf ids collide: every document must be ingested by exactly one rank")
        return cls(dim, local_rows, sum(counts[:rank]), sum(counts), leaf_ids, docstore, group=group, **kw)

    @classmethod
    def from_local_index(cls, index: HipVectorIndex, group=None, **kw) -> "ShardedHipVectorIndex":
        index._compact()
        mat, leaf_ids = index.snapshot()
        return cls.from_local(index.dim, mat.contiguous(), leaf_ids, index.docstore, group=group,
                              embed_model=kw.pop("embed_model", index.embed_model),
                              score_mode=kw.pop("score_mode", index.score_mode), **kw)

    @classmethod
    def load(cls, persist_dir: str, device=None, embed_model=None, score_mode: str = "chroma", group=None,
             **kw) -> "ShardedHipVectorIndex":
        world, rank = _world(group)
        blob, raw = _read_persisted(persist_dir, rows=lambda n_rows: slice(*_sh.shard_bounds(n_rows, world, rank)))
        n = len(blob["leaf_ids"])
        lo, hi = _sh.shard_bounds(n, world, rank)
        dev = torch.device("cuda" if device in (None, "cuda") else device)
        if dev.type == "cuda" and dev.index is None:
            dev = torch.device("cuda", torch.cuda.current_device())
        import numpy as np

        rows = torch.from_numpy(np.array(raw, copy=True)).view(torch.bfloat16).to(dev).contiguous()
        docstore = {nid: _node_from_dict(nid, d) for nid, d in blob["nodes"].items()}
        return cls(blob["dim"], rows, lo, n, blob["leaf_ids"], docstore, embed_model=embed_model, score_mode=score_mode,
                   group=group, **kw)

    @property
    def num_live(self) -> int:
        return self.n_total

    def node_score(self, cos: float) -> float:
        return math.exp(-(2.0 - 2.0 * cos)) if self.score_mode == "chroma" else cos

    def _scan_shard(self, rows: torch.Tensor, q16: torch.Tensor, k: int, base: int):
        from . import scan as _scan

        shadow = None
        if self.fp8_shadow and 0 < q16.shape[0] <= _scan.ScanShadow.MAX_QUERIES and rows.shape[0] >= _scan.ScanShadow.MIN_ROWS:
            key = rows.data_ptr()
            shadow = self._shadows.get(key)
            if shadow is None:
                with self._shadow_lock:
                    shadow = self._shadows.get(key)
                    if shadow is None:
                        shadow = self._shadows[key] = _scan.ScanShadow(rows)
        return _scan.scan_topk(rows, q16, k, idx_base=base, shadow=shadow)

    def _local_topk(self, q16: torch.Tensor, k: int):
        parts = [self._scan(rows, q16, k, base) for rows, base in self._shards]
        if len(parts) == 1:
            return parts[0]
        s = torch.cat([p[0] for p in parts], dim=1)
        i = torch.cat([p[1] for p in parts], dim=1)
        return self._merge(s, i, k)

    def _collective_topk(self, q16: torch.Tensor, k: int):
        world, rank = _world(self.group)
        err = None
        try:
            s, i = self._local_topk(q16, k)
        except Exception as exc:
            err = exc
            s = torch.zeros((q16.shape[0], k), dtype=torch.float32, device=q16.device)
            i = torch.full((q16.shape[0], k), _POISON, dtype=torch.int32, device=q16.device)
        all_s, all_i = _sh.gather_partials(s, i, self.group)
        bad = (all_i[:1, ::k] == _POISON).cpu().tolist()[0] if all_i.shape[0] else [False] * world
        if err is not None or any(bad):
            failed = [r for r, b in enumerate(bad) if b] or [rank]
            raise ShardRoundError(f"shard scan failed on rank(s) {failed}: the round's queries have no complete result") from err
        if all_s.shape[1] == k:
            return all_s, all_i
        return self._merge(all_s, all_i, k)

    def _unit_bf16(self, query_emb: torch.Tensor) -> torch.Tensor:
        q = query_emb.to(self.device, dtype=torch.float32)
        return (q / q.norm(dim=1, keepdim=True).clamp_min(1e-12)).to(torch.bfloat16).contiguous()

    def search(self, query_emb: torch.Tensor, k: int, filters=None):
        if filters is not None:
            raise NotImplementedError("metadata filters are not supported on a row-sharded index")
        q16 = self._unit_bf16(query_emb)
        world, rank = _world(self.group)
        if world == 1:
            return self._local_topk(q16, k)
        if self._tick_fronts:
            raise RuntimeError("this index is being served by a lock-step tick front (as_retriever at world > 1, "
                               "queries='partitioned'): a direct search() would interleave its collectives with the front's; "
                               "go through retrieve(), or close() the retriever first")
        with self._collective_lock:
            nq = q16.shape[0]
            if self.queries == "partitioned" and not self.ragged_queries:
                return self._round_partitioned(q16, k, nq)
            if self.queries == "partitioned":
                counts = torch.zeros(world, dtype=torch.int64, device=q16.device)
                dist.all_gather_into_tensor(counts, torch.tensor([nq], dtype=torch.int64, device=q16.device), group=self.group)
                return self._round_partitioned(q16, k, int(counts.max().item()))
            return self._collective_topk(q16, k)

    def _round_partitioned(self, q16: torch.Tensor, k: int, nmax: int):
        world, rank = _world(self.group)
        nq = q16.shape[0]
        if nmax == 0:
            return (torch.empty((0, k), dtype=torch.float32, device=q16.device),
                    torch.empty((0, k), dtype=torch.int32, device=q16.device))
        if nq < nmax:
            q16 = torch.cat([q16, torch.zeros((nmax - nq, q16.shape[1]), dtype=q16.dtype, device=q16.device)], 0)
        all_q = _sh.gather_queries(q16, self.group)
        s, i = self._collective_topk(all_q, k)
        return s[rank * nmax: rank * nmax + nq], i[rank * nmax: rank * nmax + nq]

    def as_retriever(self, similarity_top_k: int = 10, coalesce: bool = True, max_batch: int = 64,
                     max_wait_s: float = 0.0, **_kw) -> "ShardedHipVectorRetriever":
        if _kw.get("filters") is not None:
            raise NotImplementedError("metadata filters are not supported on a row-sharded index")
        if self.leaf_ids is None or self.docstore is None:
            raise ValueError("this ShardedHipVectorIndex was built without node tables (search-only)")
        world, _ = _world(self.group)
        tick = coalesce and world > 1 and self.queries == "partitioned"
        return ShardedHipVectorRetriever(self, similarity_top_k, coalesce=coalesce and world == 1, max_batch=max_batch,
                                         max_wait_s=max_wait_s, tick=tick)

    def snapshot(self):
        return None, self.leaf_ids


class _TickSlot:
    __slots__ = ("bundle", "event", "result", "error")

    def __init__(self, bundle):
        self.bundle, self.event, self.result, self.error = bundle, threading.Event(), None, None


class _TickFront:

    def __init__(self, retriever: "ShardedHipVectorRetriever", max_batch: int, idle_sleep_s: float = 2e-4, idle_sleep_max_s: float = 5e-3):
        self.retriever, self.index = retriever, retriever.index
        self.max_batch = max(1, int(max_batch))
        self.idle_sleep_s, self.idle_sleep_max_s = idle_sleep_s, max(idle_sleep_s, idle_sleep_max_s)
        self._wake = threading.Event()
        self._lock = threading.Lock()
        self._queue: List[_TickSlot] = []
        self._closing = False
        self._dead: Optional[BaseException] = None
        self.ticks = self.rounds = self.items = 0
        self.index._tick_fronts += 1
        self._thread = threading.Thread(target=self._loop, name="tt-tick-front", daemon=True)
        self._thread.start()

    def submit(self, bundle):
        slot = _TickSlot(bundle)
        with self._lock:
            if self._closing or self._dead is not None:
                raise RuntimeError("the sharded retriever's serving front is closed") from self._dead
            self._queue.append(slot)
        self._wake.set()
        slot.event.wait()
        if slot.error is not None:
            raise slot.error
        return slot.result

    def close(self, timeout: Optional[float] = None) -> None:
        with self._lock:
            self._closing = True
        self._wake.set()
        self._thread.join(timeout)

    def _embed_own(self, batch: List[_TickSlot]):
        r = self.retriever
        try:
            return batch, self.index._unit_bf16(r._query_matrix([s.bundle for s in batch]))
        except Exception as first:
            if len(batch) == 1:
                batch[0].error = first
                batch[0].event.set()
                return [], None
        good, rows = [], []
        for s in batch:
            try:
                rows.append(self.index._unit_bf16(r._query_matrix([s.bundle])))
                good.append(s)
            except Exception as exc:
                s.error = exc
                s.event.set()
        return good, (torch.cat(rows, 0) if rows else None)

    def _loop(self) -> None:
        idx, r = self.index, self.retriever
        world, rank = _world(idx.group)
        dev = idx.device
        batch: List[_TickSlot] = []
        idle_ticks = 0
        import contextlib

        ctx = contextlib.nullcontext()
        if dev.type == "cuda":
            torch.cuda.set_device(dev)
            if os.environ.get("TT_RETRIEVE_STREAM", "1") != "0" and _lib.isa_checked():
                stream = torch.cuda.Stream(device=dev, priority=-1)
                if idx._written is not None:
                    stream.wait_event(idx._written)
                ctx = torch.cuda.stream(stream)
        try:
            with ctx:
                while True:
                    with self._lock:
                        batch = self._queue[: self.max_batch]
                        del self._queue[: len(batch)]
                        closing = self._closing and not self._queue
                    q16, round_error = None, None
                    if batch:
                        batch, q16 = self._embed_own(batch)
                    nq = len(batch)
                    flags = torch.zeros((world, 2), dtype=torch.int64, device=dev)
                    with idx._collective_lock:
                        dist.all_gather_into_tensor(flags.view(-1), torch.tensor([nq, 1 if (closing and nq == 0) else 0],
                                                                                 dtype=torch.int64, device=dev), group=idx.group)
                        flags_h = flags.cpu()
                        nmax = int(flags_h[:, 0].max().item())
                        self.ticks += 1
                        if nmax == 0:
                            if bool(flags_h[:, 1].all().item()):
                                return
                            hits = None
                        else:
                            k = min(r.similarity_top_k, idx.n_total)
                            if q16 is None:
                                q16 = torch.zeros((0, idx.dim), dtype=torch.bfloat16, device=dev)
                            try:
                                hits = idx._round_partitioned(q16, k, nmax) if k >= 1 else None
                            except ShardRoundError as exc:
                                round_error, hits = exc, None
                            self.rounds += 1
                    if nmax == 0:
                        idle_ticks += 1
                        self._wake.wait(min(self.idle_sleep_max_s, self.idle_sleep_s * (1 << min(idle_ticks - 1, 10))))
                        self._wake.clear()
                        continue
                    idle_ticks = 0
                    self._wake.clear()
                    if batch and round_error is not None:
                        for s_ in batch:
                            s_.error = round_error
                            s_.event.set()
                        batch = []
                    if batch:
                        if hits is None:
                            results = [[] for _ in batch]
                        else:
                            scores, rows = hits[0].cpu().tolist(), hits[1].cpu().tolist()
                            results = [r.nodes_from_hits(s_, r_, idx.leaf_ids) for s_, r_ in zip(scores, rows)]
                        self.items += len(batch)
                        for s_, res in zip(batch, results):
                            s_.result = res
                            s_.event.set()
                        batch = []
        except BaseException as exc:
            with self._lock:
                self._dead = exc
                self._closing = True
                pending = batch + self._queue
                self._queue = []
            for s_ in pending:
                if not s_.event.is_set():
                    s_.error = RuntimeError(f"sharded serving front stopped: {exc!r}")
                    s_.event.set()
        finally:
            idx._tick_fronts -= 1


class ShardedHipVectorRetriever(HipVectorRetriever):

    def __init__(self, index, similarity_top_k: int = 10, coalesce: bool = True, max_batch: int = 64, max_wait_s: float = 0.0,
                 tick: bool = False):
        super().__init__(index, similarity_top_k, coalesce=coalesce, max_batch=max_batch, max_wait_s=max_wait_s)
        self._tick = _TickFront(self, max_batch) if tick else None

    def retrieve(self, query) -> List[NodeWithScore]:
        if self._tick is not None:
            from .schema import as_query_bundle

            return self._tick.submit(as_query_bundle(query))
        return super().retrieve(query)

    _retrieve = retrieve

    def close(self, timeout: Optional[float] = None) -> None:
        if self._tick is not None:
            self._tick.close(timeout)

    def _retrieve_batch(self, bundles) -> List[List[NodeWithScore]]:
        idx = self.index
        k = min(self.similarity_top_k, idx.n_total)
        if k < 1:
            return [[] for _ in bundles]
        world, _ = _world(idx.group)
        stream = self._gpu_stream() if world == 1 and idx.device.type == "cuda" else None
        if stream is None:
            scores, rows = idx.search(self._query_matrix(bundles), k)
            scores, rows = scores.cpu().tolist(), rows.cpu().tolist()
        else:
            with torch.cuda.stream(stream):
                if idx._written is not None:
                    stream.wait_event(idx._written)
                scores, rows = idx.search(self._query_matrix(bundles), k)
                scores, rows = scores.cpu().tolist(), rows.cpu().tolist()
        return [self.nodes_from_hits(s, r, idx.leaf_ids) for s, r in zip(scores, rows)]
```

tensor-truth_amd/vector_index.py:

```python
from __future__ import annotations

import json
import logging
import math
import os
import re
import threading
from datetime import datetime, timezone
from typing import Dict, Iterable, List, Optional, Sequence

import numpy as np
import torch

from . import _lib
from . import scan as _scan
from . import metadata_filter as _mf
from .coalesce import Coalescer
from .schema import MetadataMode, NodeWithScore, TextNode, as_query_bundle

logger = logging.getLogger(__name__)

INDEX_METADATA_FILENAME = "index_metadata.json"
INDEX_VERSION = "1.0"


def sanitize_model_id(model_name: str) -> str:
    name = model_name.split("/")[-1].lower()
    name = re.sub(r"[^a-z0-9\-_.]", "-", name)
    return re.sub(r"-+", "-", name).strip("-")


class HipVectorIndex:
    def __init__(self, dim: int, device=None, embed_model=None, score_mode: str = "chroma"):
        dev = torch.device("cuda" if device in (None, "cuda") else device)
        if dev.type != "cuda":
            raise RuntimeError("HipVectorIndex needs a HIP device; tensor_truth_amd has no CPU path")
        if dev.index is None:
            dev = torch.device("cuda", torch.cuda.current_device())
        if dim % 128 or dim > 1024:
            raise ValueError(f"dim {dim}: the scan kernels take multiples of 128 up to 1024")
        self.dim, self.device = dim, dev
        self.embed_model = embed_model
        self.score_mode = score_mode
        self._mat = torch.empty((0, dim), dtype=torch.bfloat16, device=dev)
        self.n = 0
        self.leaf_ids: List[str] = []
        self.leaf_token_ids: Optional[Dict[str, np.ndarray]] = None
        self.leaf_token_origin: Optional[tuple] = None
        self.docstore: Dict[str, TextNode] = {}
        self.ref_docs: Dict[str, List[str]] = {}
        self._lock = threading.RLock()
        self._version = 0
        self._dead = 0
        self._row_of: Optional[Dict[str, int]] = None
        self._written: Optional[torch.cuda.Event] = None
        self.fp8_shadow = os.environ.get("TT_SCAN_SHADOW", "1") != "0"
        self._shadow = None
        self._cols: Dict[str, _mf.CodeColumn] = {}
        self._generation = 0

    def _mark_written(self) -> None:
        ev = torch.cuda.Event()
        ev.record(torch.cuda.current_stream(self.device))
        self._written = ev

    def _reserve(self, n_new: int) -> None:
        need = self.n + n_new
        if need > self._mat.shape[0]:
            cap = max(need, 2 * self._mat.shape[0], 1024)
            grown = torch.empty((cap, self.dim), dtype=torch.bfloat16, device=self.device)
            grown[: self.n] = self._mat[: self.n]
            self._mat = grown
            for col in self._cols.values():
                col.reserve(cap)

    def add(self, nodes: Sequence[TextNode], embeddings=None, show_progress: bool = False, token_ids=None) -> List[str]:
        if not nodes:
            return []
        if embeddings is None:
            if self.embed_model is None:
                raise ValueError("no embeddings given and the index has no embed_model")
            texts = [n.get_content(metadata_mode=MetadataMode.EMBED) for n in nodes]
            if hasattr(self.embed_model, "_embed_texts"):
                emb = self.embed_model._embed_texts(texts, getattr(self.embed_model, "text_instruction", ""))
            else:
                emb = torch.tensor(self.embed_model.get_text_embedding_batch(texts, show_progress=show_progress))
        else:
            emb = embeddings if torch.is_tensor(embeddings) else torch.tensor(np.asarray(embeddings, dtype=np.float32))
        if emb.shape != (len(nodes), self.dim):
            raise ValueError(f"embeddings {tuple(emb.shape)} != ({len(nodes)}, {self.dim})")
        emb = emb.to(self.device, dtype=torch.float32)
        emb = emb / emb.norm(dim=1, keepdim=True).clamp_min(1e-12)
        with self._lock:
            self._reserve(len(nodes))
            self._mat[self.n:self.n + len(nodes)] = emb.to(torch.bfloat16)
            for key, col in self._cols.items():
                col.append(_mf.VOCAB.key(key).codes(_mf.metadata_values({nd.id_: nd for nd in nodes}, [nd.id_ for nd in nodes], key)))
            self._mark_written()
            for j, nd in enumerate(nodes):
                self.leaf_ids.append(nd.id_)
                self.docstore[nd.id_] = nd
                if self._row_of is not None:
                    self._row_of[nd.id_] = self.n + j
            if token_ids is not None:
                origin = self._embedder_token_origin()
                if self.leaf_token_ids and self.leaf_token_origin is not None and origin != self.leaf_token_origin:
                    logger.warning("index: leaf token ids dropped (the embedder's tokenizer or text instruction changed between adds)")
                    self.leaf_token_ids = None
                if self.leaf_token_ids is None:
                    self.leaf_token_ids = {}
                self.leaf_token_origin = origin
                limit = getattr(self.embed_model, "max_length", None)
                for nd, ids in zip(nodes, token_ids):
                    if limit is None or len(ids) < limit:
                        self.leaf_token_ids[nd.id_] = np.asarray(ids[1:-1], dtype=np.int32)
                    else:
                        self.leaf_token_ids.pop(nd.id_, None)
            elif self.leaf_token_ids:
                for nd in nodes:
                    self.leaf_token_ids.pop(nd.id_, None)
            self.n += len(nodes)
            self._version += 1
        return [nd.id_ for nd in nodes]

    def _embedder_token_origin(self):
        em = self.embed_model
        if em is None or not hasattr(em, "_tokenizer"):
            return None
        from .tokenization import tokenizer_signature

        return tokenizer_signature(em._tokenizer), getattr(em, "text_instruction", "") or ""

    def token_source(self):
        if not self.leaf_token_ids or self.leaf_token_origin is None:
            return None
        return self.leaf_token_ids.get, self.leaf_token_origin[0], self.leaf_token_origin[1]

    def add_to_docstore(self, nodes: Iterable[TextNode]) -> None:
        with self._lock:
            for nd in nodes:
                self.docstore.setdefault(nd.id_, nd)

    def delete(self, node_ids: Iterable[str]) -> int:
        drop = set(node_ids)
        with self._lock:
            if self._row_of is None:
                self._row_of = {nid: i for i, nid in enumerate(self.leaf_ids) if nid is not None}
            rows = [self._row_of.pop(nid) for nid in drop if nid in self._row_of]
            if rows:
                idx = torch.tensor(rows, dtype=torch.long, device=self.device)
                self._mat[: self.n].index_fill_(0, idx, float("nan"))
                self._mark_written()
                self._shadow = None
                for r in rows:
                    self.leaf_ids[r] = None
                self._dead += len(rows)
                self._version += 1
                if self._dead > max(1024, self.n // 4):
                    self._compact()
            for nid in drop:
                self.docstore.pop(nid, None)
                if self.leaf_token_ids is not None:
                    self.leaf_token_ids.pop(nid, None)
        return len(rows)

    def _compact(self) -> None:
        with self._lock:
            if not self._dead:
                return
            keep = [i for i, nid in enumerate(self.leaf_ids) if nid is not None]
            idx = torch.tensor(keep, dtype=torch.long, device=self.device)
            self._mat = self._mat[: self.n].index_select(0, idx) if keep else torch.empty(
                (0, self.dim), dtype=torch.bfloat16, device=self.device)
            self._cols = {key: _mf.CodeColumn.from_device(key, self.device, col.dev[: self.n].index_select(0, idx))
                          for key, col in self._cols.items()}
            self._generation += 1
            self._mark_written()
            self.leaf_ids = [self.leaf_ids[i] for i in keep]
            self.n, self._dead, self._row_of = len(keep), 0, None
            self._version += 1

    @property
    def num_live(self) -> int:
        return self.n - self._dead

    @property
    def matrix(self) -> torch.Tensor:
        return self._mat[: self.n]

    def snapshot(self):
        with self._lock:
            return _Snapshot((self._mat[: self.n], self.leaf_ids), self._generation)

    def _column(self, key: str, snapshot=None) -> "_mf.CodeColumn":
        with self._lock:
            rows = self.n if snapshot is None else int(snapshot[0].shape[0])
            gen = getattr(snapshot, "generation", None) if snapshot is not None else self._generation
            if gen == self._generation and rows <= self.n:
                col = self._cols.get(key)
                if col is None:
                    codes = _mf.VOCAB.key(key).codes(_mf.metadata_values(self.docstore, self.leaf_ids[: self.n], key))
                    col = self._cols[key] = _mf.CodeColumn(key, self.device, codes, cap=self._mat.shape[0])
                return col
            ids = list(snapshot[1][:rows])
            docstore = self.docstore
        if len(ids) < rows:
            raise ValueError(f"snapshot holds {rows} rows but {len(ids)} leaf ids")
        codes = _mf.VOCAB.key(key).codes(_mf.metadata_values(docstore, ids, key))
        return _mf.CodeColumn(key, self.device, codes)

    def _filtered(self, snap, q16: torch.Tensor, k: int, filters, host: bool):
        mat = snap[0]
        cf = _mf.compile_filter(filters, lambda key: self._column(key, snap), mat.shape[0], self.device)
        rows, offs = _scan.filter_rows(cf, mat.shape[0], self.device)
        if host:
            return _scan.scan_topk_rows_host(mat, q16, k, rows, offs, cf.bound)
        return _scan.scan_topk_rows(mat, q16, k, rows, offs, cf.bound)

    def _unit_bf16(self, query_emb: torch.Tensor) -> torch.Tensor:
        q = query_emb.to(self.device, dtype=torch.float32)
        return (q / q.norm(dim=1, keepdim=True).clamp_min(1e-12)).to(torch.bfloat16).contiguous()

    def _shadow_for(self, mat: torch.Tensor, n_queries: int):
        if not self.fp8_shadow or not (0 < n_queries <= _scan.ScanShadow.MAX_QUERIES) or mat.shape[0] < _scan.ScanShadow.MIN_ROWS:
            return None
        with self._lock:
            if mat.data_ptr() != self._mat.data_ptr() or mat.shape[0] > self.n:
                return None
            sh = self._shadow
            if self._written is not None and (sh is None or sh.rows < self.n):
                torch.cuda.current_stream(self.device).wait_event(self._written)
            if sh is None or sh.base_ptr != self._mat.data_ptr() or sh.cap_rows < self.n:
                sh = self._shadow = _scan.ScanShadow(self._mat[: self.n], cap_rows=self._mat.shape[0])
                sh.base_ptr = self._mat.data_ptr()
            elif sh.rows < self.n:
                sh.extend(self._mat, self.n)
            return sh if sh.rows >= mat.shape[0] else None

    def search(self, query_emb: torch.Tensor, k: int, snapshot=None, filters=None):
        snap = snapshot if snapshot is not None else self.snapshot()
        mat = snap[0]
        if _mf.filter_key(filters) is not None:
            return self._filtered(snap, self._unit_bf16(query_emb), k, filters, host=False)
        return _scan.scan_topk(mat, self._unit_bf16(query_emb), k, shadow=self._shadow_for(mat, query_emb.shape[0]))

    def search_host(self, query_emb: torch.Tensor, k: int, snapshot=None, filters=None):
        snap = snapshot if snapshot is not None else self.snapshot()
        mat = snap[0]
        if _mf.filter_key(filters) is not None:
            return self._filtered(snap, self._unit_bf16(query_emb), k, filters, host=True)
        return _scan.scan_topk_host(mat, self._unit_bf16(query_emb), k, shadow=self._shadow_for(mat, query_emb.shape[0]))

    def node_score(self, cos: float) -> float:
        return math.exp(-(2.0 - 2.0 * cos)) if self.score_mode == "chroma" else cos

    def as_retriever(self, similarity_top_k: int = 10, coalesce: bool = True, max_batch: int = 64,
                     max_wait_s: float = 0.0, filters=None, **_kw) -> "HipVectorRetriever":
        return HipVectorRetriever(self, similarity_top_k, coalesce=coalesce, max_batch=max_batch, max_wait_s=max_wait_s,
                                  filters=filters)

    def persist(self, persist_dir: str, embedding_model: Optional[str] = None, chunk_sizes=None,
                chunking_strategy: Optional[str] = None, chunk_overlap: Optional[int] = None) -> None:
        os.makedirs(persist_dir, exist_ok=True)
        with _persist_guard(persist_dir):
            with self._lock:
                self._compact()
                mat_host = self.matrix.cpu().view(torch.int16).numpy()
                leaf_ids = list(self.leaf_ids)
                nodes = {nid: _node_to_dict(nd) for nid, nd in self.docstore.items()}
                ref_docs = {k: list(v) for k, v in self.ref_docs.items()}
                n_rows = self.n
                tok = None
                if self.leaf_token_ids:
                    arrs = [self.leaf_token_ids.get(nid) for nid in leaf_ids]
                    lens = np.fromiter((0 if a is None else len(a) for a in arrs), dtype=np.int32, count=len(arrs))
                    flat = np.concatenate([a for a in arrs if a is not None and len(a)]) if int(lens.sum()) else np.zeros(0, np.int32)
                    tok = (flat.astype(np.int32), lens)
                tok_origin = self.leaf_token_origin
            gen = _next_generation(persist_dir)
            corpus_name = f"corpus.{gen}.bf16"
            if tok is not None and tok_origin is None:
                logger.warning("index: leaf token ids not persisted (the tokenizer they came from is unknown)")
                tok = None
            tokens_name = f"leaf_tokens.{gen}.npz" if tok is not None else None

            def _atomic(name: str, write) -> None:
                tmp = os.path.join(persist_dir, f".{name}.tmp.{os.getpid()}.{threading.get_ident()}")
                write(tmp)
                os.replace(tmp, os.path.join(persist_dir, name))

            _atomic(corpus_name, lambda t: mat_host.tofile(t))
            if tok is not None:
                def _write_tokens(t):
                    with open(t, "wb") as f:
                        np.savez(f, flat=tok[0], lens=tok[1])
                _atomic(tokens_name, _write_tokens)
            model = embedding_model or getattr(self.embed_model, "model_name", None)
            meta = {"embedding_model": model, "embedding_model_id": sanitize_model_id(model) if model else None,
                    "created_at": datetime.now(timezone.utc).isoformat(), "index_version": INDEX_VERSION,
                    "chunk_sizes": list(chunk_sizes) if chunk_sizes is not None else None, "chunk_overlap": chunk_overlap,
                    "chunking_strategy": chunking_strategy,
                    "embedding_dim": self.dim, "num_vectors": n_rows, "store": f"tensor_truth_amd/{corpus_name}"}

            def _dump(obj):
                def w(t):
                    with open(t, "w") as f:
                        json.dump(obj, f)
                return w

            _atomic(INDEX_METADATA_FILENAME, _dump(meta))
            _atomic("nodes.json", _dump({"dim": self.dim, "leaf_ids": leaf_ids, "nodes": nodes, "ref_docs": ref_docs,
                                         "corpus_file": corpus_name, "generation": gen, "leaf_tokens_file": tokens_name,
                                         "leaf_tokens_tokenizer": tok_origin[0] if tokens_name else None,
                                         "leaf_tokens_instruction": tok_origin[1] if tokens_name else None}))
            for name in os.listdir(persist_dir):
                g = _generation_of(name)
                if g is None and name.startswith("leaf_tokens.") and name.endswith(".npz"):
                    try:
                        g = int(name[len("leaf_tokens."):-len(".npz")])
                    except ValueError:
                        g = None
                if g is not None and g < gen:
                    try:
                        os.remove(os.path.join(persist_dir, name))
                    except OSError:
                        pass

    @classmethod
    def load(cls, persist_dir: str, device=None, embed_model=None, score_mode: str = "chroma") -> "HipVectorIndex":
        blob, raw = _read_persisted(persist_dir)
        idx = cls(blob["dim"], device, embed_model, score_mode)
        idx._mat = torch.from_numpy(np.array(raw, copy=True)).view(torch.bfloat16).to(idx.device).contiguous()
        idx._mark_written()
        idx.n = raw.shape[0]
        idx.leaf_ids = list(blob["leaf_ids"])
        idx.ref_docs = {k: list(v) for k, v in (blob.get("ref_docs") or {}).items()}
        idx.docstore = {nid: _node_from_dict(nid, d) for nid, d in blob["nodes"].items()}
        tname = blob.get("leaf_tokens_file")
        if tname and os.path.exists(os.path.join(persist_dir, tname)):
            sig, instr = blob.get("leaf_tokens_tokenizer"), blob.get("leaf_tokens_instruction")
            mine = idx._embedder_token_origin()
            if sig is None or instr is None:
                logger.warning("index %s: leaf token ids ignored (persisted without the tokenizer signature they were made with)", persist_dir)
            elif mine is not None and mine != (sig, instr):
                logger.warning("index %s: leaf token ids ignored (tokenised with %s / instruction %r at ingest, loaded next to %s / %r)",
                               persist_dir, sig, instr, mine[0], mine[1])
            else:
                with np.load(os.path.join(persist_dir, tname)) as z:
                    flat, lens = z["flat"], z["lens"]
                if len(lens) == len(idx.leaf_ids):
                    ends = np.cumsum(lens)
                    idx.leaf_token_ids = {nid: flat[e - n:e] for nid, e, n in zip(idx.leaf_ids, ends, lens) if n > 0 and nid is not None}
                    idx.leaf_token_origin = (sig, instr)
        return idx


class _Snapshot(tuple):

    def __new__(cls, pair, generation: int):
        t = super().__new__(cls, pair)
        t.generation = generation
        return t


_LINK_KEYS = ("parent_id", "child_ids", "prev_id", "next_id")
_CONTENT_KEYS = ("excluded_embed_metadata_keys", "excluded_llm_metadata_keys", "metadata_template",
                 "metadata_separator", "text_template")


def _node_to_dict(nd) -> dict:
    d = {"text": nd.text, "metadata": nd.metadata}
    for key in _LINK_KEYS:
        v = getattr(nd, key, None)
        d[key] = list(v or []) if key == "child_ids" else v
    for key in _CONTENT_KEYS:
        v = getattr(nd, key, None)
        if v:
            d[key] = list(v) if isinstance(v, (list, tuple)) else v
    return d


def _copy_node_attrs(src, dst, keys) -> None:
    for key in keys:
        if hasattr(src, key):
            v = getattr(src, key)
            try:
                setattr(dst, key, list(v) if isinstance(v, (list, tuple)) else v)
            except Exception:
                pass


def _node_from_dict(nid: str, d: dict):
    nd = TextNode(text=d["text"], id_=nid, metadata=d["metadata"])
    for key in _LINK_KEYS + _CONTENT_KEYS:
        if key in d or key in _LINK_KEYS:
            v = d.get(key)
            try:
                setattr(nd, key, list(v or []) if key in ("child_ids", "excluded_embed_metadata_keys",
                                                          "excluded_llm_metadata_keys") else v)
            except Exception:
                pass
    return nd


def _generation_of(name: str):
    if name.startswith("corpus.") and name.endswith(".bf16"):
        try:
            return int(name[len("corpus."):-len(".bf16")])
        except ValueError:
            return None
    return None


def _next_generation(persist_dir: str) -> int:
    gen = 0
    try:
        with open(os.path.join(persist_dir, "nodes.json")) as f:
            gen = int(json.load(f).get("generation", 0))
    except (OSError, ValueError):
        pass
    try:
        for name in os.listdir(persist_dir):
            g = _generation_of(name)
            if g is not None:
                gen = max(gen, g)
    except OSError:
        pass
    return gen + 1


_PERSIST_LOCKS: dict = {}
_PERSIST_LOCKS_GUARD = threading.Lock()


class _persist_guard:

    def __init__(self, persist_dir: str):
        self.path = os.path.realpath(persist_dir)
        with _PERSIST_LOCKS_GUARD:
            self.lock = _PERSIST_LOCKS.setdefault(self.path, threading.Lock())
        self.fh = None

    def __enter__(self):
        self.lock.acquire()
        try:
            import fcntl

            self.fh = open(os.path.join(self.path, ".persist.lock"), "a+")
            fcntl.flock(self.fh, fcntl.LOCK_EX)
        except (ImportError, OSError):
            if self.fh is not None:
                self.fh.close()
                self.fh = None
        return self

    def __exit__(self, *exc):
        try:
            if self.fh is not None:
                import fcntl

                fcntl.flock(self.fh, fcntl.LOCK_UN)
                self.fh.close()
        finally:
            self.lock.release()
        return False


def _read_persisted(persist_dir: str, rows=None):
    for attempt in range(3):
        with open(os.path.join(persist_dir, "nodes.json")) as f:
            blob = json.load(f)
        path = os.path.join(persist_dir, blob.get("corpus_file", "corpus.bf16"))
        n, dim = len(blob["leaf_ids"]), blob["dim"]
        try:
            if os.path.getsize(path) != n * dim * 2:
                raise ValueError(f"{path} and nodes.json disagree on the number of rows")
            raw = np.memmap(path, dtype=np.int16, mode="r", shape=(n, dim)) if n else np.zeros((0, dim), np.int16)
            break
        except FileNotFoundError:
            if attempt == 2:
                raise
    if callable(rows):
        rows = rows(n)
    return blob, (raw[rows] if rows is not None else raw)


class HipVectorRetriever:

    def __init__(self, index: HipVectorIndex, similarity_top_k: int = 10, coalesce: bool = True, max_batch: int = 64,
                 max_wait_s: float = 0.0, filters=None):
        self.index = index
        self.similarity_top_k = similarity_top_k
        self.filters = filters
        self.filter_key = _mf.filter_key(filters)
        self._front = Coalescer(self._retrieve_batch, max_batch, max_wait_s) if coalesce else None
        self._stream: Optional[torch.cuda.Stream] = None

    def _gpu_stream(self):
        if os.environ.get("TT_RETRIEVE_STREAM", "1") == "0":
            return None
        if not _lib.isa_checked():
            if not getattr(HipVectorRetriever, "_warned_isa", False):
                HipVectorRetriever._warned_isa = True
                logger.warning("libtt_hip.so carries no valid ISA-check stamp (csrc/check_isa.py): retrieval stays on the caller's stream")
            return None
        if self._stream is None:
            dev = self.index.device
            self._stream = torch.cuda.Stream(device=dev, priority=-1)
        return self._stream

    def retrieve(self, query) -> List[NodeWithScore]:
        qb = as_query_bundle(query)
        if self.index.num_live == 0:
            return []
        if self._front is not None:
            return self._front.submit(qb)
        return self._retrieve_batch([qb])[0]

    def _query_matrix(self, bundles) -> torch.Tensor:
        idx = self.index
        strs, owner = [], []
        for i, qb in enumerate(bundles):
            if getattr(qb, "embedding", None) is None:
                ss = list(qb.embedding_strs)
                strs += ss
                owner += [i] * len(ss)
        rows: List[Optional[torch.Tensor]] = [None] * len(bundles)
        if strs:
            em = idx.embed_model
            if em is None:
                raise ValueError("retriever needs an embed_model or a QueryBundle with an embedding")
            if hasattr(em, "query_embedding_device"):
                E = em.query_embedding_device(strs).to(idx.device, dtype=torch.float32)
            else:
                E = torch.tensor([em.get_agg_embedding_from_queries([s]) for s in strs], dtype=torch.float32,
                                 device=idx.device)
            if len(strs) == len(set(owner)):
                for j, i in enumerate(owner):
                    rows[i] = E[j]
            else:
                for i in sorted(set(owner)):
                    sel = [j for j, o in enumerate(owner) if o == i]
                    rows[i] = E[sel].mean(dim=0)
        for i, qb in enumerate(bundles):
            if rows[i] is None:
                rows[i] = torch.tensor(qb.embedding, dtype=torch.float32, device=idx.device)
        return torch.stack(rows, 0)

    def _retrieve_batch(self, bundles) -> List[List[NodeWithScore]]:
        idx = self.index
        snap = idx.snapshot()
        mat, leaf_ids = snap
        k = min(self.similarity_top_k, max(idx.num_live, 0), mat.shape[0])
        if k < 1:
            return [[] for _ in bundles]
        stream = self._gpu_stream()
        fkw = {} if self.filter_key is None else {"filters": self.filters}
        if stream is None:
            scores, rows = idx.search_host(self._query_matrix(bundles), k, snapshot=snap, **fkw)
            scores, rows = scores.tolist(), rows.tolist()
        else:
            written = getattr(idx, "_written", None)
            with torch.cuda.stream(stream):
                if written is not None:
                    stream.wait_event(written)
                scores, rows = idx.search_host(self._query_matrix(bundles), k, snapshot=snap, **fkw)
                scores, rows = scores.tolist(), rows.tolist()
        return [self.nodes_from_hits(s, r, leaf_ids) for s, r in zip(scores, rows)]

    def nodes_from_hits(self, scores: Sequence[float], rows: Sequence[int], leaf_ids=None) -> List[NodeWithScore]:
        idx = self.index
        ids = idx.leaf_ids if leaf_ids is None else leaf_ids
        out = []
        for s, r in zip(scores, rows):
            if r < 0 or r >= len(ids):
                continue
            src = idx.docstore.get(ids[r]) if ids[r] is not None else None
            if src is None:
                continue
            node = TextNode(text=src.text, id_=src.id_, metadata=dict(src.metadata))
            _copy_node_attrs(src, node, _LINK_KEYS + _CONTENT_KEYS)
            out.append(NodeWithScore(node=node, score=float(idx.node_score(s))))
        return out

    _retrieve = retrieve


class HipIndexGroup:

    def __init__(self, indexes: Sequence[HipVectorIndex]):
        if not indexes:
            raise ValueError("HipIndexGroup needs at least one index")
        if len({(ix.dim, ix.device) for ix in indexes}) != 1:
            raise ValueError("grouped indexes must share embedding width and device")
        self.indexes = list(indexes)
        self.dim, self.device = indexes[0].dim, indexes[0].device
        self._lock = threading.RLock()
        self._stamp = None
        self._mat = None
        self._leaf_ids: List[list] = []
        self.offsets: List[int] = []
        self.fp8_shadow = os.environ.get("TT_SCAN_SHADOW", "1") != "0"
        self._seg_shadows: Dict[int, object] = {}
        self._packed_cols: Dict[str, object] = {}

    def _pack(self) -> None:
        for ix in self.indexes:
            ix._lock.acquire()
        try:
            stamp = tuple((ix._version, ix.n) for ix in self.indexes)
            if stamp == self._stamp:
                return
            offs = [0]
            for ix in self.indexes:
                offs.append(offs[-1] + ix.n)
            mat = torch.empty((offs[-1], self.dim), dtype=torch.bfloat16, device=self.device)
            for ix, lo in zip(self.indexes, offs):
                mat[lo:lo + ix.n] = ix._mat[: ix.n]
                ix._mat = mat[lo:lo + ix.n]
                ix._mark_written()
            self._mat, self.offsets, self._stamp = mat, offs, stamp
            self._leaf_ids = [ix.leaf_ids for ix in self.indexes]
            self._seg_shadows = {}
            self._packed_cols = {}
        finally:
            for ix in self.indexes:
                ix._lock.release()

    def _snapshot_for(self, q: torch.Tensor, k: int):
        S = _scan.ScanShadow
        with self._lock:
            self._pack()
            mat, offs, ids = self._mat, list(self.offsets), list(self._leaf_ids)
            shadows = None
            big = [m for m, (lo, hi) in enumerate(zip(offs, offs[1:])) if hi - lo >= max(S.MIN_ROWS, 128 * k)]
            if self.fp8_shadow and 0 < q.shape[0] <= S.MAX_QUERIES and big:
                for m in big:
                    if m not in self._seg_shadows:
                        self._seg_shadows[m] = S(mat[offs[m]:offs[m + 1]])
                shadows = dict(self._seg_shadows)
        return mat, offs, ids, shadows

    @staticmethod
    def _scan_modules(mat, offs, q, k, shadows) -> torch.Tensor:
        nq, n_seg = q.shape[0], len(offs) - 1
        packed = torch.empty((n_seg, 2 * nq * k + 1), dtype=torch.int32, device=mat.device)
        for m, (lo, hi) in enumerate(zip(offs, offs[1:])):
            _scan.scan_topk(mat[lo:hi], q, k, _packed=packed[m], shadow=shadows.get(m))
        return packed

    @staticmethod
    def _unpack_modules(packed: torch.Tensor, mat, offs, q, k):
        nq, n_seg = q.shape[0], len(offs) - 1
        s = packed[:, : nq * k].view(torch.float32).view(n_seg, nq, k).permute(1, 0, 2).contiguous()
        r = packed[:, nq * k: 2 * nq * k].view(n_seg, nq, k).permute(1, 0, 2).contiguous()
        for m in torch.nonzero(packed[:, -1].cpu()).flatten().tolist():
            es, er = _scan.scan_topk(mat[offs[m]:offs[m + 1]], q, k, exact_dense=True)
            s[:, m], r[:, m] = es.to(s.device), er.to(r.device)
        return s, r

    def _packed_column(self, key: str):
        col = self._packed_cols.get(key)
        if col is None:
            parts = [ix._column(key) for ix in self.indexes]
            codes = torch.cat([c.dev[: ix.n] for c, ix in zip(parts, self.indexes)]) if self.indexes else None
            width = max(len(c.counts) for c in parts)
            counts = np.zeros(width, np.int64)
            for c in parts:
                counts[: len(c.counts)] += c.counts
            col = self._packed_cols[key] = _mf.CodeColumn.from_device(key, self.device, codes, counts)
        return col

    def _filtered_search(self, q: torch.Tensor, k: int, filters, host: bool):
        with self._lock:
            self._pack()
            for ix in self.indexes:
                ix._lock.acquire()
            try:
                if tuple((ix._version, ix.n) for ix in self.indexes) != self._stamp:
                    self._pack()
                mat, offs, ids = self._mat, list(self.offsets), list(self._leaf_ids)
                cf = _mf.compile_filter(filters, self._packed_column, offs[-1], self.device)
            finally:
                for ix in self.indexes:
                    ix._lock.release()
        rows, loff = _scan.filter_rows(cf, mat.shape[0], self.device, seg_offsets=offs)
        if host:
            s, r = _scan.scan_topk_rows_host(mat, q, k, rows, loff, cf.bound, seg_offsets=offs)
        else:
            s, r = _scan.scan_topk_rows(mat, q, k, rows, loff, cf.bound, seg_offsets=offs)
        return s, r, ids

    def search(self, query_emb: torch.Tensor, k: int, return_snapshot: bool = False, filters=None):
        q = query_emb.to(self.device, dtype=torch.float32)
        q = (q / q.norm(dim=1, keepdim=True).clamp_min(1e-12)).to(torch.bfloat16).contiguous()
        if _mf.filter_key(filters) is not None:
            s, r, ids = self._filtered_search(q, k, filters, host=False)
            return (s, r, ids) if return_snapshot else (s, r)
        mat, offs, ids, shadows = self._snapshot_for(q, k)
        if shadows is None:
            s, r = _scan.scan_topk_segmented(mat, q, k, offs)
        else:
            s, r = self._unpack_modules(self._scan_modules(mat, offs, q, k, shadows), mat, offs, q, k)
        return (s, r, ids) if return_snapshot else (s, r)

    def search_host(self, query_emb: torch.Tensor, k: int, filters=None):
        q = query_emb.to(self.device, dtype=torch.float32)
        q = (q / q.norm(dim=1, keepdim=True).clamp_min(1e-12)).to(torch.bfloat16).contiguous()
        if _mf.filter_key(filters) is not None:
            return self._filtered_search(q, k, filters, host=True)
        mat, offs, ids, shadows = self._snapshot_for(q, k)
        if shadows is None:
            s, r = _scan.scan_topk_segmented(mat, q, k, offs)
            return s.cpu(), r.cpu(), ids
        s, r = self._unpack_modules(self._scan_modules(mat, offs, q, k, shadows).cpu(), mat, offs, q, k)
        return s, r, ids
```

Baseline: 114.7.

## Extend fp8 shadow prefilter to batches of up to 32 queries with tightening pass

Raises the fp8 shadow prefilter limit from 4 to 32 queries per call. For batches it keeps per-survivor upper bounds, rescores a provisional top-k exactly, and then tightens the survivor table before the final bf16 rescore. The per-query rescore and select launches are folded into single launches that use one grid row per query. Batched workloads that previously fell back to the full bf16 scan should now take the shadow path, at the cost of extra kernels, a larger workspace and more shadow-lifecycle handling.

```diff
diff --git a/tensor-truth_amd/csrc/scan.h b/tensor-truth_amd/csrc/scan.h
--- a/tensor-truth_amd/csrc/scan.h
+++ b/tensor-truth_amd/csrc/scan.h
@@ -21,6 +21,7 @@
     int prof_id;
     const int32_t* row_table;
     const int32_t* row_cnt;
+    int64_t table_stride;
     const int32_t* gather_rows;
     const int32_t* row_range;
 };
diff --git a/tensor-truth_amd/csrc/scan.hip b/tensor-truth_amd/csrc/scan.hip
--- a/tensor-truth_amd/csrc/scan.hip
+++ b/tensor-truth_amd/csrc/scan.hip
@@ -101,7 +101,19 @@
     const int wave = __builtin_amdgcn_readfirstlane(tid >> 6);
     char* scratch = smem + C::kQImageBytes + wave * kScratchPerWave;
 
-    const int q0 = blockIdx.y * kBM;
+    int q0 = blockIdx.y * kBM;
+    if constexpr (OUT == 1 && (MODE == 0 || G)) {
+        if (p.table_stride != 0) {
+            const int y = blockIdx.y;
+            q0 = 0;
+            p.queries += (size_t)y * D;
+            p.n_queries = 1;
+            if constexpr (G) p.gather_rows += (size_t)y * p.table_stride;
+            else p.row_table += (size_t)y * p.table_stride;
+            p.row_cnt += y;
+            p.dense += (size_t)y * p.dense_stride;
+        }
+    }
 
     {
         constexpr int kPiecesPerRow = D / 8;
@@ -141,8 +153,9 @@
     }
     const int32_t* gtab = nullptr;
     if constexpr (G) {
-        const int32_t b = p.row_range[0];
-        const int64_t n = (int64_t)p.row_range[1] - b;
+        const bool per_query = OUT == 1 && p.table_stride != 0;
+        const int32_t b = per_query ? 0 : p.row_range[0];
+        const int64_t n = per_query ? (int64_t)*p.row_cnt : (int64_t)p.row_range[1] - b;
         const int64_t span = p.row_hi - p.row_lo;
         p.row_hi = p.row_lo + (n < 0 ? 0 : (n < span ? n : span));
         gtab = p.gather_rows + b;
@@ -346,7 +359,7 @@
 static int launch_d(const ScanParams& p, int mode, int out, int blocks, int q_tiles, hipStream_t stream) {
     const int load_mode = mode & 15;
     const int var = mode >> 4;
-    if (p.row_range) {
+    if (p.row_range || (p.gather_rows && p.table_stride != 0)) {
         switch (out) {
             case 0: return launch_one<D, 1, 0, 0, true>(p, blocks, q_tiles, stream);
             case 1: return launch_one<D, 1, 1, 0, true>(p, blocks, q_tiles, stream);
@@ -381,7 +394,15 @@
 }
 
 int tt_scan_launch(const ScanParams& p, int dim, int mode, int out, int blocks, hipStream_t stream) {
-    const int q_tiles = (p.n_queries + kBM - 1) / kBM;
+    int q_tiles = (p.n_queries + kBM - 1) / kBM;
+    if (p.table_stride != 0) {
+        const bool lines = p.gather_rows && !p.row_table && !p.row_range;
+        if (!p.row_cnt || out != 1 || !(lines || (p.row_table && !p.gather_rows && (mode & 15) == 0))) {
+            tt_set_error("scan: per-query tables need a gather path (row_table in mode 0, or gather_rows) and dense scores");
+            return TT_E_INVALID;
+        }
+        q_tiles = p.n_queries;
+    }
     if (p.row_hi <= p.row_lo || q_tiles == 0) return TT_OK;
     const int64_t n_groups = (p.row_hi - p.row_lo + 31) / 32;
     const int64_t max_blocks = out != 0 ? n_groups : (n_groups + kWaves - 1) / kWaves;
diff --git a/tensor-truth_amd/csrc/scan_api.hip b/tensor-truth_amd/csrc/scan_api.hip
--- a/tensor-truth_amd/csrc/scan_api.hip
+++ b/tensor-truth_amd/csrc/scan_api.hip
@@ -168,44 +168,64 @@
     return l;
 }
 struct ShadowPlan {
+    bool batch;
     int64_t n0, stride;
     int blocks, n_waves, capw, cap;
-    size_t off_sample, off_ss, off_si, off_thr, off_planes, off_qinfo, off_list, off_wcnt, off_table, off_tcnt, off_dense, total;
+    int cap2, kpad;
+    size_t off_sample, off_ss, off_si, off_thr, off_planes, off_qinfo, off_list, off_wcnt, off_table, off_tub, off_tcnt, off_kcnt, off_kdense,
+        off_table2, off_tcnt2, off_dense, total;
 };
 ShadowPlan shadow_plan(int64_t n_rows, int dim, int n_queries, int k, int cus) {
     ShadowPlan pl{};
+    pl.batch = n_queries > kShadowLoneQueries;
     int64_t n0 = kSampleRows;
     if (n0 < (int64_t)128 * k) n0 = (int64_t)128 * k;
     if (n0 < n_rows / 32) n0 = n_rows / 32 / 32 * 32;
     pl.n0 = n0 < n_rows ? n0 : n_rows;
     pl.stride = ((pl.n0 + 31) / 32 + 31) / 32 * 32;
+    const int wpb = kShadowWavesPerBlock;
     pl.blocks = cus > 0 ? cus : 256;
     const int64_t groups = (n_rows + 15) / 16;
-    if ((int64_t)pl.blocks * kShadowWavesPerBlock > groups) pl.blocks = (int)((groups + kShadowWavesPerBlock - 1) / kShadowWavesPerBlock);
+    if ((int64_t)pl.blocks * wpb > groups) pl.blocks = (int)((groups + wpb - 1) / wpb);
     if (pl.blocks < 1) pl.blocks = 1;
-    pl.n_waves = pl.blocks * kShadowWavesPerBlock;
+    pl.n_waves = pl.blocks * wpb;
     int64_t cap = n_rows / 16;
     if (cap < 65536) cap = 65536;
     if (cap > (1 << 20)) cap = 1 << 20;
     if (cap > (n_rows + 31) / 32 * 32) cap = (n_rows + 31) / 32 * 32;
     pl.cap = (int)((cap + 31) / 32 * 32);
-    int64_t capw = 4 * (int64_t)pl.cap / pl.n_waves;
+    int64_t capw = (pl.batch ? 2 : 4) * (int64_t)pl.cap / pl.n_waves;
     if (capw < 64) capw = 64;
     pl.capw = (int)capw;
+    int64_t cap2 = n_rows / 64;
+    if (cap2 < 8192) cap2 = 8192;
+    if (cap2 > pl.cap) cap2 = pl.cap;
+    pl.cap2 = (int)((cap2 + 31) / 32 * 32);
+    pl.kpad = (k + 31) / 32 * 32;
     const int qpad = 64;
+    const size_t entry = pl.batch ? sizeof(int2) : sizeof(int32_t);
     size_t off = 0;
     auto take = [&](size_t bytes) { size_t o = off; off += tt_align_up(bytes, 256); return o; };
     pl.off_sample = take((size_t)qpad * pl.stride * sizeof(float));
     pl.off_ss = take((size_t)qpad * k * sizeof(float));
     pl.off_si = take((size_t)qpad * k * sizeof(int32_t));
     pl.off_thr = take((size_t)qpad * sizeof(float));
-    pl.off_planes = take((size_t)(dim / 128) * 4 * 1024);
+    pl.off_planes = take((size_t)tt_shadow_column_groups(n_queries) * (dim / 128) * 4 * 1024);
     pl.off_qinfo = take(32 * sizeof(float));
-    pl.off_list = take((size_t)n_queries * pl.n_waves * pl.capw * sizeof(int32_t));
+    pl.off_list = take((size_t)n_queries * pl.n_waves * pl.capw * entry);
     pl.off_wcnt = take((size_t)n_queries * pl.n_waves * sizeof(int32_t));
     pl.off_table = take((size_t)n_queries * pl.cap * sizeof(int32_t));
     pl.off_tcnt = take((size_t)qpad * sizeof(int32_t));
-    pl.off_dense = take((size_t)pl.cap * sizeof(float));
+    if (pl.batch) {
+        pl.off_tub = take((size_t)n_queries * pl.cap * sizeof(float));
+        pl.off_kcnt = take((size_t)qpad * sizeof(int32_t));
+        pl.off_kdense = take((size_t)n_queries * pl.kpad * sizeof(float));
+        pl.off_table2 = take((size_t)n_queries * pl.cap2 * sizeof(int32_t));
+        pl.off_tcnt2 = take((size_t)qpad * sizeof(int32_t));
+        pl.off_dense = take((size_t)n_queries * pl.cap2 * sizeof(float));
+    } else {
+        pl.off_dense = take((size_t)n_queries * pl.cap * sizeof(float));
+    }
     pl.total = off;
     return pl;
 }
@@ -514,10 +534,29 @@
 }
 
 size_t tt_scan_shadow_workspace_bytes(int64_t n_rows, int dim, int n_queries, int k) {
-    if (n_rows <= 0 || n_queries <= 0 || n_queries > 4 || k < 1 || dim <= 0 || dim % 128) return 0;
+    if (n_rows <= 0 || n_queries <= 0 || n_queries > kShadowMaxQueries || k < 1 || dim <= 0 || dim % 128) return 0;
     int cus = tt_cu_count_cached();
     if (cus <= 0) cus = 256;
     return shadow_plan(n_rows, dim, n_queries, k, cus).total;
+}
+
+static int shadow_rescore(const void* corpus, const void* queries, int n_queries, int dim, const int32_t* table, int64_t table_stride,
+                          const int32_t* cnt, int64_t bound, float* dense, int64_t dense_stride, bool lines, int cus, hipStream_t st) {
+    ScanParams rp{};
+    rp.corpus = (const uint16_t*)corpus;
+    rp.queries = (const uint16_t*)queries;
+    rp.row_lo = 0;
+    rp.row_hi = bound;
+    rp.n_queries = n_queries;
+    rp.dense = dense;
+    rp.dense_stride = dense_stride;
+    if (lines) rp.gather_rows = table;
+    else rp.row_table = table;
+    rp.row_cnt = cnt;
+    rp.table_stride = table_stride;
+    rp.prof_id = TT_K_SCAN_TAIL;
+    const int blocks = cus / n_queries > 0 ? cus / n_queries : 1;
+    return tt_scan_launch(rp, dim, lines ? 1 : 0, 1, blocks, st);
 }
 
 int tt_scan_topk_shadow(const void* corpus_bf16, const void* shadow, int64_t cap_rows, int64_t n_rows, int dim, const void* queries_bf16,
@@ -526,7 +565,8 @@
     int rc = check_common(corpus_bf16, n_rows, dim, queries_bf16, n_queries, k, out_scores, out_idx);
     if (rc) return rc;
     if (n_queries == 0) return TT_OK;
-    TT_CHECK_ARG(n_queries <= 4, "n_queries=%d: the shadow prefilter serves lone callers (<= 4 queries per call)", n_queries);
+    TT_CHECK_ARG(n_queries <= kShadowMaxQueries, "n_queries=%d: the shadow prefilter serves batches of up to %d queries per call", n_queries,
+                 kShadowMaxQueries);
     TT_CHECK_ARG(shadow && ((uintptr_t)shadow % 256) == 0 && n_rows <= cap_rows, "shadow missing, misaligned or smaller than n_rows");
     TT_CHECK_ARG(n_rows >= (int64_t)128 * k && n_rows > 8192, "n_rows=%lld: shards this small take tt_scan_topk's dense path", (long long)n_rows);
     hipStream_t st = (hipStream_t)stream;
@@ -542,6 +582,8 @@
     char* ws = (char*)workspace;
     float* sample = (float*)(ws + pl.off_sample);
     float* thr = (float*)(ws + pl.off_thr);
+    float* ss = (float*)(ws + pl.off_ss);
+    int32_t* si = (int32_t*)(ws + pl.off_si);
     const int mode = scan_mode_from_env();
     ScanParams sp{};
     sp.corpus = (const uint16_t*)corpus_bf16;
@@ -561,8 +603,8 @@
     s1.m_fixed = (int)((pl.n0 + 31) / 32);
     s1.cap = INT_MAX;
     s1.k = k;
-    s1.out_scores = (float*)(ws + pl.off_ss);
-    s1.out_idx = (int32_t*)(ws + pl.off_si);
+    s1.out_scores = ss;
+    s1.out_idx = si;
     s1.out_stride = k;
     s1.thr_out = thr;
     rc = tt_select_launch(s1, n_queries, st);
@@ -571,46 +613,66 @@
     const char* sb = (const char*)shadow;
     uint16_t* planes = (uint16_t*)(ws + pl.off_planes);
     float* qinfo = (float*)(ws + pl.off_qinfo);
-    int32_t* list = (int32_t*)(ws + pl.off_list);
+    void* list = ws + pl.off_list;
     int32_t* wcnt = (int32_t*)(ws + pl.off_wcnt);
     int32_t* table = (int32_t*)(ws + pl.off_table);
     int32_t* tcnt = (int32_t*)(ws + pl.off_tcnt);
+    float* dense = (float*)(ws + pl.off_dense);
     rc = tt_shadow_query_launch((const uint16_t*)queries_bf16, n_queries, dim, planes, qinfo, st);
     if (rc) return rc;
     rc = tt_shadow_filter_launch((const uint8_t*)sb, (const float*)(sb + l.off_be), (const float*)(sb + l.off_dn), n_rows, dim, planes, qinfo, thr,
-                                 n_queries, pl.blocks, list, wcnt, pl.capw, status_flag, st);
-    if (rc) return rc;
-    rc = tt_shadow_compact_launch(list, wcnt, pl.n_waves, pl.capw, n_queries, table, pl.cap, tcnt, status_flag, st);
-    if (rc) return rc;
-    float* dense = (float*)(ws + pl.off_dense);
-    for (int q = 0; q < n_queries; ++q) {
-        ScanParams rp{};
-        rp.corpus = (const uint16_t*)corpus_bf16;
-        rp.queries = (const uint16_t*)queries_bf16 + (size_t)q * dim;
-        rp.row_lo = 0;
-        rp.row_hi = pl.cap;
-        rp.n_queries = 1;
-        rp.dense = dense;
-        rp.dense_stride = pl.cap;
-        rp.row_table = table + (size_t)q * pl.cap;
-        rp.row_cnt = tcnt + q;
-        rp.prof_id = TT_K_SCAN_TAIL;
-        rc = tt_scan_launch(rp, dim, 0, 1, cus, st);
+                                 n_queries, pl.blocks, list, pl.batch, wcnt, pl.capw, status_flag, st);
+    if (rc) return rc;
+    const int32_t* final_table = table;
+    const int32_t* final_cnt = tcnt;
+    int final_cap = pl.cap;
+    if (!pl.batch) {
+        rc = tt_shadow_compact_launch(list, false, wcnt, pl.n_waves, pl.capw, n_queries, table, nullptr, pl.cap, tcnt, nullptr, status_flag, st);
         if (rc) return rc;
-        SelectParams s2{};
-        s2.scores = dense;
-        s2.idx = table + (size_t)q * pl.cap;
-        s2.stride = pl.cap;
-        s2.cnt = tcnt + q;
-        s2.cap = pl.cap;
-        s2.k = k;
-        s2.out_scores = out_scores + (size_t)q * k;
-        s2.out_idx = out_idx + (size_t)q * k;
-        s2.out_stride = k;
-        s2.overflow_flag = status_flag;
-        rc = tt_select_launch(s2, 1, st);
+    } else {
+        float* tub = (float*)(ws + pl.off_tub);
+        int32_t* kcnt = (int32_t*)(ws + pl.off_kcnt);
+        float* kdense = (float*)(ws + pl.off_kdense);
+        int32_t* table2 = (int32_t*)(ws + pl.off_table2);
+        int32_t* tcnt2 = (int32_t*)(ws + pl.off_tcnt2);
+        rc = tt_shadow_compact_launch(list, true, wcnt, pl.n_waves, pl.capw, n_queries, table, tub, pl.cap, tcnt, tcnt2, status_flag, st);
         if (rc) return rc;
-    }
+        SelectParams su{};
+        su.scores = tub;
+        su.idx = table;
+        su.stride = pl.cap;
+        su.cnt = tcnt;
+        su.cap = pl.cap;
+        su.k = k;
+        su.out_scores = ss;
+        su.out_idx = si;
+        su.out_stride = k;
+        su.cnt_out = kcnt;
+        rc = tt_select_launch(su, n_queries, st);
+        if (rc) return rc;
+        rc = shadow_rescore(corpus_bf16, queries_bf16, n_queries, dim, si, k, kcnt, k, kdense, pl.kpad, true, cus, st);
+        if (rc) return rc;
+        rc = tt_shadow_tighten_launch(table, tub, tcnt, pl.cap, thr, kdense, pl.kpad, kcnt, k, n_queries, 32, table2, pl.cap2, tcnt2, st);
+        if (rc) return rc;
+        final_table = table2;
+        final_cnt = tcnt2;
+        final_cap = pl.cap2;
+    }
+    rc = shadow_rescore(corpus_bf16, queries_bf16, n_queries, dim, final_table, final_cap, final_cnt, final_cap, dense, final_cap, pl.batch, cus, st);
+    if (rc) return rc;
+    SelectParams s2{};
+    s2.scores = dense;
+    s2.idx = final_table;
+    s2.stride = final_cap;
+    s2.cnt = final_cnt;
+    s2.cap = final_cap;
+    s2.k = k;
+    s2.out_scores = out_scores;
+    s2.out_idx = out_idx;
+    s2.out_stride = k;
+    s2.overflow_flag = status_flag;
+    rc = tt_select_launch(s2, n_queries, st);
+    if (rc) return rc;
     if (idx_base != 0) {
         const int n = n_queries * k;
         hipLaunchKernelGGL(add_idx_base_kernel, dim3((n + 255) / 256), dim3(256), 0, st, out_idx, n, idx_base);
diff --git a/tensor-truth_amd/csrc/shadow.h b/tensor-truth_amd/csrc/shadow.h
--- a/tensor-truth_amd/csrc/shadow.h
+++ b/tensor-truth_amd/csrc/shadow.h
@@ -1,11 +1,17 @@
 #pragma once
 #include "common.h"
 
+constexpr int kShadowMaxQueries = 32;
+constexpr int kShadowLoneQueries = 4;
 constexpr int kShadowWavesPerBlock = 8;
+inline int tt_shadow_column_groups(int n_queries) { return n_queries > 16 ? 2 : 1; }
 int tt_shadow_build_launch(const uint16_t* corpus, int64_t n_rows, int dim, uint8_t* shadow, float* be, float* dn, hipStream_t st);
 int tt_shadow_query_launch(const uint16_t* queries, int n_queries, int dim, uint16_t* frags, float* qinfo, hipStream_t st);
 int tt_shadow_filter_launch(const uint8_t* shadow, const float* be, const float* dn, int64_t n_rows, int dim, const uint16_t* frags,
-                            const float* qinfo, const float* thr, int n_queries, int blocks, int32_t* list, int32_t* wave_cnt, int capw,
-                            int32_t* status_flag, hipStream_t st);
-int tt_shadow_compact_launch(const int32_t* list, const int32_t* wave_cnt, int n_waves, int capw, int n_queries, int32_t* table, int cap,
-                             int32_t* table_cnt, int32_t* status_flag, hipStream_t st);
+                            const float* qinfo, const float* thr, int n_queries, int blocks, void* list, bool with_ub, int32_t* wave_cnt,
+                            int capw, int32_t* status_flag, hipStream_t st);
+int tt_shadow_compact_launch(const void* list, bool with_ub, const int32_t* wave_cnt, int n_waves, int capw, int n_queries, int32_t* table,
+                             float* table_ub, int cap, int32_t* table_cnt, int32_t* zero_cnt, int32_t* status_flag, hipStream_t st);
+int tt_shadow_tighten_launch(const int32_t* table, const float* table_ub, const int32_t* table_cnt, int cap, const float* thr,
+                             const float* kscores, int kstride, const int32_t* kcnt, int k, int n_queries, int slices, int32_t* table2,
+                             int cap2, int32_t* cnt2, hipStream_t st);
diff --git a/tensor-truth_amd/csrc/shadow.hip b/tensor-truth_amd/csrc/shadow.hip
--- a/tensor-truth_amd/csrc/shadow.hip
+++ b/tensor-truth_amd/csrc/shadow.hip
@@ -47,6 +47,7 @@
 
 __global__ __launch_bounds__(64) void shadow_query_kernel(const uint16_t* queries, int n_queries, int dim, uint16_t* frags, float* qinfo) {
     const int q = blockIdx.x, lane = threadIdx.x;
+    const int g = q >> 4, j = q & 15, nkt = dim >> 7;
     float sq = 0.f;
     for (int c = lane; c < dim; c += 64) {
         uint16_t v = 0;
@@ -54,7 +55,7 @@
         const float x = bf16_to_f32(v);
         sq = fmaf(x, x, sq);
         const int kt = c >> 7, g4 = (c & 127) >> 5, f = (c & 31) >> 3, e = c & 7;
-        frags[((size_t)(kt * 4 + f) * 64 + (g4 * 16 + q)) * 8 + e] = v;
+        frags[((size_t)((g * nkt + kt) * 4 + f) * 64 + (g4 * 16 + j)) * 8 + e] = v;
     }
     sq = wave_sum(sq);
     if (lane == 0) qinfo[q] = sqrtf(sq) * 1.0005f + 1e-9f;
@@ -69,7 +70,7 @@
     const float* thr;
     int64_t n_rows;
     int n_queries;
-    int32_t* list;
+    void* list;
     int32_t* wave_cnt;
     int capw;
     int32_t* status_flag;
@@ -81,25 +82,32 @@
     return __builtin_amdgcn_perm(__float_as_uint(f[1]), __float_as_uint(f[0]), 0x07060302u);
 }
 
-template <int D>
+template <int D, int NG, bool UB>
 __global__ __launch_bounds__(kSThreads, 2) void shadow_filter_kernel(ShadowParams p) {
     constexpr int NKT = D / 128;
+    constexpr int kWaves = kSWaves, kThreads = kSThreads, kQ = 16 * NG;
+    constexpr int kFragBytes = NG * NKT * 4 * 1024;
     extern __shared__ __attribute__((aligned(16))) char smem[];
     uint4* qf = reinterpret_cast<uint4*>(smem);
-    int* lcnt = reinterpret_cast<int*>(smem + NKT * 4 * 1024);
+    int* lcnt = reinterpret_cast<int*>(smem + kFragBytes);
     const int tid = threadIdx.x, lane = tid & 63;
     const int wave = __builtin_amdgcn_readfirstlane(tid >> 6);
-    char* scratch = smem + NKT * 4 * 1024 + kSWaves * 16 * sizeof(int) + wave * 2048;
-    for (int i = tid; i < NKT * 4 * 64; i += kSThreads) qf[i] = reinterpret_cast<const uint4*>(p.frags)[i];
-    if (tid < kSWaves * 16) lcnt[tid] = 0;
+    char* scratch = smem + kFragBytes + kWaves * kQ * sizeof(int) + wave * 2048;
+    for (int i = tid; i < NG * NKT * 4 * 64; i += kThreads) qf[i] = reinterpret_cast<const uint4*>(p.frags)[i];
+    for (int i = tid; i < kWaves * kQ; i += kThreads) lcnt[i] = 0;
     __syncthreads();
 
     const int j = lane & 15, g4 = lane >> 4;
-    const bool qok = j < p.n_queries;
-    const float thr = qok ? p.thr[j] : __builtin_inff();
-    const float qn = p.qinfo[j];
-    const int n_waves = gridDim.x * kSWaves;
-    const int wg = blockIdx.x * kSWaves + wave;
+    bool qok[NG];
+    float thr[NG], qn[NG];
+#pragma unroll
+    for (int g = 0; g < NG; ++g) {
+        qok[g] = 16 * g + j < p.n_queries;
+        thr[g] = qok[g] ? p.thr[16 * g + j] : __builtin_inff();
+        qn[g] = p.qinfo[16 * g + j];
+    }
+    const int n_waves = gridDim.x * kWaves;
+    const int wg = blockIdx.x * kWaves + wave;
     const int64_t n_groups = (p.n_rows + 15) / 16;
     typedef unsigned int u32x4 __attribute__((ext_vector_type(4)));
     const int lrow = lane >> 3, lpiece = lane & 7;
@@ -121,7 +129,9 @@
         }
     };
     auto process = [&](const u32x4 (&a)[NKT][2], int64_t grp) {
-        f32x4 acc = f32x4{0.f, 0.f, 0.f, 0.f};
+        f32x4 acc[NG];
+#pragma unroll
+        for (int g = 0; g < NG; ++g) acc[g] = f32x4{0.f, 0.f, 0.f, 0.f};
 #pragma unroll
         for (int kt = 0; kt < NKT; ++kt) {
             *reinterpret_cast<u32x4*>(scratch + woff0) = a[kt][0];
@@ -133,8 +143,11 @@
                 const uint32_t w0 = (f < 2 ? x0 : x1)[(f & 1) * 2], w1 = (f < 2 ? x0 : x1)[(f & 1) * 2 + 1];
                 const uint4 av = make_uint4(e4m3x2_to_bf16x2<false>(w0), e4m3x2_to_bf16x2<true>(w0), e4m3x2_to_bf16x2<false>(w1),
                                             e4m3x2_to_bf16x2<true>(w1));
-                const uint4 bv = qf[(kt * 4 + f) * 64 + lane];
-                acc = TT_MFMA_16x16x32(__builtin_bit_cast(ex8, av), __builtin_bit_cast(ex8, bv), acc);
+#pragma unroll
+                for (int g = 0; g < NG; ++g) {
+                    const uint4 bv = qf[((g * NKT + kt) * 4 + f) * 64 + lane];
+                    acc[g] = TT_MFMA_16x16x32(__builtin_bit_cast(ex8, av), __builtin_bit_cast(ex8, bv), acc[g]);
+                }
             }
         }
         const int64_t r0 = grp * 16 + g4 * 4;
@@ -144,13 +157,19 @@
         const float dns[4] = {dn4.x, dn4.y, dn4.z, dn4.w};
         constexpr float kGamma2 = 2.0f * (float)(D + 8) * 1.1920928955078125e-7f;
 #pragma unroll
-        for (int r = 0; r < 4; ++r) {
-            const float ub = acc[r] * (1.0f / kShadowScale) + qn * bes[r] + (kGamma2 * qn * (dns[r] + bes[r]) + 1e-30f);
-            if (qok && ub >= thr && r0 + r < p.n_rows) {
-                const int pos = atomicAdd(&lcnt[wave * 16 + j], 1);
-                if (pos < p.capw) p.list[((size_t)j * n_waves + wg) * p.capw + pos] = (int32_t)(r0 + r);
+        for (int g = 0; g < NG; ++g)
+#pragma unroll
+            for (int r = 0; r < 4; ++r) {
+                const float ub = acc[g][r] * (1.0f / kShadowScale) + qn[g] * bes[r] + (kGamma2 * qn[g] * (dns[r] + bes[r]) + 1e-30f);
+                if (qok[g] && ub >= thr[g] && r0 + r < p.n_rows) {
+                    const int pos = atomicAdd(&lcnt[wave * kQ + 16 * g + j], 1);
+                    if (pos < p.capw) {
+                        const size_t slot = ((size_t)(16 * g + j) * n_waves + wg) * p.capw + pos;
+                        if constexpr (UB) reinterpret_cast<int2*>(p.list)[slot] = make_int2((int32_t)(r0 + r), __float_as_int(ub));
+                        else reinterpret_cast<int32_t*>(p.list)[slot] = (int32_t)(r0 + r);
+                    }
+                }
             }
-        }
     };
 
     u32x4 a0[NKT][2], a1[NKT][2];
@@ -168,7 +187,7 @@
     asm volatile("s_waitcnt lgkmcnt(0)" ::: "memory");
     __builtin_amdgcn_wave_barrier();
     if (lane < p.n_queries) {
-        const int c = reinterpret_cast<volatile int*>(lcnt)[wave * 16 + lane];
+        const int c = reinterpret_cast<volatile int*>(lcnt)[wave * kQ + lane];
         p.wave_cnt[(size_t)lane * n_waves + wg] = c < p.capw ? c : p.capw;
         if (c > p.capw && p.status_flag) atomicOr(p.status_flag, 2);
     }
@@ -214,6 +233,129 @@
     }
 }
 
+__global__ __launch_bounds__(1024) void shadow_compact_ub_kernel(const int2* list, const int32_t* wave_cnt, int n_waves, int capw, int32_t* table,
+                                                                 float* table_ub, int cap, int32_t* table_cnt, int32_t* zero_cnt,
+                                                                 int32_t* status_flag) {
+    extern __shared__ int offs[];
+    __shared__ int wsum[16];
+    __shared__ int total;
+    const int q = blockIdx.x, tid = threadIdx.x, lane = tid & 63, wv = tid >> 6;
+    const int32_t* cnts = wave_cnt + (size_t)q * n_waves;
+    const int per = (n_waves + 1023) / 1024;
+    int mine = 0;
+    for (int i = 0; i < per; ++i) {
+        const int w = tid * per + i;
+        if (w < n_waves) mine += cnts[w];
+    }
+    int inc = mine;
+#pragma unroll
+    for (int o = 1; o < 64; o <<= 1) {
+        const int v = __shfl_up(inc, o, 64);
+        if (lane >= o) inc += v;
+    }
+    if (lane == 63) wsum[wv] = inc;
+    __syncthreads();
+    int base = 0;
+    for (int i = 0; i < wv; ++i) base += wsum[i];
+    if (tid == 1023) total = base + inc;
+    int off = base + inc - mine;
+    for (int i = 0; i < per; ++i) {
+        const int w = tid * per + i;
+        if (w >= n_waves) break;
+        offs[w] = off;
+        off += cnts[w];
+    }
+    __syncthreads();
+    const int nw = gridDim.y * 16;
+    int32_t* trow = table + (size_t)q * cap;
+    float* tub = table_ub + (size_t)q * cap;
+    for (int w0 = (blockIdx.y * 16 + wv) * 4; w0 < n_waves; w0 += nw * 4) {
+        int c[4], o[4];
+        int2 v[4];
+#pragma unroll
+        for (int u = 0; u < 4; ++u) {
+            const int w = w0 + u;
+            c[u] = w < n_waves ? cnts[w] : 0;
+            o[u] = w < n_waves ? offs[w] : 0;
+        }
+#pragma unroll
+        for (int u = 0; u < 4; ++u)
+            if (lane < c[u]) v[u] = list[((size_t)q * n_waves + w0 + u) * capw + lane];
+#pragma unroll
+        for (int u = 0; u < 4; ++u) {
+            if (lane < c[u] && o[u] + lane < cap) {
+                trow[o[u] + lane] = v[u].x;
+                tub[o[u] + lane] = __int_as_float(v[u].y);
+            }
+            for (int e = lane + 64; e < c[u]; e += 64) {
+                if (o[u] + e >= cap) break;
+                const int2 x = list[((size_t)q * n_waves + w0 + u) * capw + e];
+                trow[o[u] + e] = x.x;
+                tub[o[u] + e] = __int_as_float(x.y);
+            }
+        }
+    }
+    if (blockIdx.y == 0 && tid == 0) {
+        zero_cnt[q] = 0;
+        table_cnt[q] = total < cap ? total : cap;
+        if (total > cap && status_flag) atomicOr(status_flag, 4);
+    }
+}
+
+__global__ __launch_bounds__(256) void shadow_tighten_kernel(const int32_t* table, const float* table_ub, const int32_t* table_cnt, int cap,
+                                                             const float* thr, const float* kscores, int kstride, const int32_t* kcnt, int k,
+                                                             int32_t* table2, int cap2, int32_t* cnt2) {
+    constexpr int kIt = 4;
+    const int q = blockIdx.x, lane = threadIdx.x & 63;
+    const int gw = blockIdx.y * 4 + (threadIdx.x >> 6), nw = gridDim.y * 4;
+    float t = thr[q];
+    if (kcnt[q] >= k) {
+        float mn = __builtin_inff();
+        bool bad = false;
+        for (int i = lane; i < k; i += 64) {
+            const float s = kscores[(size_t)q * kstride + i];
+            bad = bad || s != s;
+            mn = fminf(mn, s);
+        }
+#pragma unroll
+        for (int o = 32; o > 0; o >>= 1) mn = fminf(mn, __shfl_xor(mn, o, 64));
+        if (__builtin_amdgcn_ballot_w64(bad) == 0ull && mn > t) t = mn;
+    }
+    const int n = table_cnt[q];
+    const unsigned long long below = (1ull << lane) - 1ull;
+    for (int base = gw * 64 * kIt; base < n; base += nw * 64 * kIt) {
+        bool keep[kIt];
+        int32_t row[kIt];
+        unsigned long long mask[kIt];
+#pragma unroll
+        for (int u = 0; u < kIt; ++u) {
+            const int i = base + u * 64 + lane;
+            keep[u] = false;
+            row[u] = -1;
+            if (i < n) {
+                keep[u] = table_ub[(size_t)q * cap + i] >= t;
+                row[u] = table[(size_t)q * cap + i];
+            }
+        }
+        int found = 0;
+#pragma unroll
+        for (int u = 0; u < kIt; ++u) {
+            mask[u] = __builtin_amdgcn_ballot_w64(keep[u]);
+            found += __builtin_popcountll(mask[u]);
+        }
+        if (found == 0) continue;
+        int start = 0;
+        if (lane == 0) start = atomicAdd(&cnt2[q], found);
+        start = __shfl(start, 0, 64);
+#pragma unroll
+        for (int u = 0; u < kIt; ++u) {
+            const int pos = start + __builtin_popcountll(mask[u] & below);
+            if (keep[u] && pos < cap2) table2[(size_t)q * cap2 + pos] = row[u];
+            start += __builtin_popcountll(mask[u]);
+        }
+    }
+}
+
 }
 
 int tt_shadow_build_launch(const uint16_t* corpus, int64_t n_rows, int dim, uint8_t* shadow, float* be, float* dn, hipStream_t st) {
@@ -224,48 +366,81 @@
 }
 
 int tt_shadow_query_launch(const uint16_t* queries, int n_queries, int dim, uint16_t* frags, float* qinfo, hipStream_t st) {
-    hipLaunchKernelGGL(shadow_query_kernel, dim3(16), dim3(64), 0, st, queries, n_queries, dim, frags, qinfo);
+    hipLaunchKernelGGL(shadow_query_kernel, dim3(16 * tt_shadow_column_groups(n_queries)), dim3(64), 0, st, queries, n_queries, dim, frags, qinfo);
     TT_CHECK_LAUNCH();
     return TT_OK;
 }
 
-template <int D>
+template <int D, int NG, bool UB>
 static int launch_filter(const ShadowParams& p, int blocks, hipStream_t st) {
-    constexpr size_t lds = (D / 128) * 4 * 1024 + kSWaves * 16 * sizeof(int) + kSWaves * 2048;
-    TT_SET_MAX_LDS(shadow_filter_kernel<D>, lds);
+    constexpr int waves = kSWaves;
+    constexpr size_t lds = (size_t)NG * (D / 128) * 4 * 1024 + waves * 16 * NG * sizeof(int) + waves * 2048;
+    static_assert(lds <= 160 * 1024, "shadow filter: fragments + scratch beyond a CU's LDS");
+    auto kern = shadow_filter_kernel<D, NG, UB>;
+    TT_SET_MAX_LDS(kern, lds);
     {
         TtProfScope prof(TT_K_SCAN_FILTER, st);
-        hipLaunchKernelGGL(shadow_filter_kernel<D>, dim3(blocks), dim3(kSThreads), lds, st, p);
+        hipLaunchKernelGGL(kern, dim3(blocks), dim3(kSThreads), lds, st, p);
     }
     TT_CHECK_LAUNCH();
     return TT_OK;
 }
 
+template <int D>
+static int launch_filter_d(const ShadowParams& p, bool with_ub, int blocks, hipStream_t st) {
+    if (!with_ub) return launch_filter<D, 1, false>(p, blocks, st);
+    if (p.n_queries <= 16) return launch_filter<D, 1, true>(p, blocks, st);
+    return launch_filter<D, 2, true>(p, blocks, st);
+}
+
 int tt_shadow_filter_launch(const uint8_t* shadow, const float* be, const float* dn, int64_t n_rows, int dim, const uint16_t* frags,
-                            const float* qinfo, const float* thr, int n_queries, int blocks, int32_t* list, int32_t* wave_cnt, int capw,
-                            int32_t* status_flag, hipStream_t st) {
+                            const float* qinfo, const float* thr, int n_queries, int blocks, void* list, bool with_ub, int32_t* wave_cnt,
+                            int capw, int32_t* status_flag, hipStream_t st) {
+    if (n_queries < 1 || n_queries > 32 || (!with_ub && n_queries > 16)) {
+        tt_set_error("shadow scan: %d queries in one filter pass", n_queries);
+        return TT_E_INVALID;
+    }
     ShadowParams p{};
     p.shadow = shadow; p.be = be; p.dn = dn; p.frags = frags; p.qinfo = qinfo; p.thr = thr; p.n_rows = n_rows; p.n_queries = n_queries;
     p.list = list; p.wave_cnt = wave_cnt; p.capw = capw; p.status_flag = status_flag;
     switch (dim) {
-        case 128: return launch_filter<128>(p, blocks, st);
-        case 256: return launch_filter<256>(p, blocks, st);
-        case 384: return launch_filter<384>(p, blocks, st);
-        case 512: return launch_filter<512>(p, blocks, st);
-        case 640: return launch_filter<640>(p, blocks, st);
-        case 768: return launch_filter<768>(p, blocks, st);
-        case 896: return launch_filter<896>(p, blocks, st);
-        case 1024: return launch_filter<1024>(p, blocks, st);
+        case 128: return launch_filter_d<128>(p, with_ub, blocks, st);
+        case 256: return launch_filter_d<256>(p, with_ub, blocks, st);
+        case 384: return launch_filter_d<384>(p, with_ub, blocks, st);
+        case 512: return launch_filter_d<512>(p, with_ub, blocks, st);
+        case 640: return launch_filter_d<640>(p, with_ub, blocks, st);
+        case 768: return launch_filter_d<768>(p, with_ub, blocks, st);
+        case 896: return launch_filter_d<896>(p, with_ub, blocks, st);
+        case 1024: return launch_filter_d<1024>(p, with_ub, blocks, st);
         default:
             tt_set_error("shadow scan: dim %d not in the compiled set {128, 256, ..., 1024}", dim);
             return TT_E_UNSUPPORTED;
     }
 }
 
-int tt_shadow_compact_launch(const int32_t* list, const int32_t* wave_cnt, int n_waves, int capw, int n_queries, int32_t* table, int cap,
-                             int32_t* table_cnt, int32_t* status_flag, hipStream_t st) {
+int tt_shadow_compact_launch(const void* list, bool with_ub, const int32_t* wave_cnt, int n_waves, int capw, int n_queries, int32_t* table,
+                             float* table_ub, int cap, int32_t* table_cnt, int32_t* zero_cnt, int32_t* status_flag, hipStream_t st) {
+    if (with_ub && n_waves > 8192) {
+        tt_set_error("shadow scan: %d survivor lists per query", n_waves);
+        return TT_E_UNSUPPORTED;
+    }
     TtProfScope prof(TT_K_SELECT, st);
-    hipLaunchKernelGGL(shadow_compact_kernel, dim3(n_queries), dim3(1024), 0, st, list, wave_cnt, n_waves, capw, table, cap, table_cnt, status_flag);
+    if (with_ub)
+        hipLaunchKernelGGL(shadow_compact_ub_kernel, dim3(n_queries, 8), dim3(1024), (size_t)n_waves * sizeof(int), st, (const int2*)list, wave_cnt,
+                           n_waves, capw, table, table_ub, cap, table_cnt, zero_cnt, status_flag);
+    else
+        hipLaunchKernelGGL(shadow_compact_kernel, dim3(n_queries), dim3(1024), 0, st, (const int32_t*)list, wave_cnt, n_waves, capw, table, cap,
+                           table_cnt, status_flag);
     TT_CHECK_LAUNCH();
     return TT_OK;
 }
+
+int tt_shadow_tighten_launch(const int32_t* table, const float* table_ub, const int32_t* table_cnt, int cap, const float* thr,
+                             const float* kscores, int kstride, const int32_t* kcnt, int k, int n_queries, int slices, int32_t* table2,
+                             int cap2, int32_t* cnt2, hipStream_t st) {
+    TtProfScope prof(TT_K_SELECT, st);
+    hipLaunchKernelGGL(shadow_tighten_kernel, dim3(n_queries, slices), dim3(256), 0, st, table, table_ub, table_cnt, cap, thr, kscores, kstride,
+                       kcnt, k, table2, cap2, cnt2);
+    TT_CHECK_LAUNCH();
+    return TT_OK;
+}
diff --git a/tensor-truth_amd/scan.py b/tensor-truth_amd/scan.py
--- a/tensor-truth_amd/scan.py
+++ b/tensor-truth_amd/scan.py
@@ -1,11 +1,14 @@
 from __future__ import annotations
 
+import logging
 import threading
 from typing import Optional, Tuple
 
 import torch
 
 from . import _lib
+
+_log = logging.getLogger(__name__)
 
 
 def _require_cuda(t: torch.Tensor, name: str) -> None:
@@ -32,6 +35,14 @@
 _ws = _Workspace()
 
 
+def build_shadow(corpus: torch.Tensor, cap_rows: Optional[int] = None, what: str = "matrix"):
+    try:
+        return ScanShadow(corpus, cap_rows=cap_rows)
+    except (RuntimeError, MemoryError) as exc:
+        _log.warning("fp8 shadow of %s (%d x %d) not built, bf16 scan instead: %s", what, corpus.shape[0], corpus.shape[1], exc)
+        return None
+
+
 def _stream_ptr(device: torch.device) -> int:
     return torch.cuda.current_stream(device).cuda_stream
 
@@ -39,7 +50,7 @@
 class ScanShadow:
 
     MIN_ROWS = 1 << 20
-    MAX_QUERIES = 4
+    MAX_QUERIES = 32
 
     def __init__(self, corpus: torch.Tensor, cap_rows: Optional[int] = None):
         _require_cuda(corpus, "corpus")
@@ -55,6 +66,7 @@
         self.ptr = (self._raw.data_ptr() + 255) // 256 * 256
         self.rows = 0
         self.base_ptr = corpus.data_ptr()
+        self.matrix = corpus
         self.ready = torch.cuda.Event()
         self.extend(corpus, int(corpus.shape[0]))
 
diff --git a/tensor-truth_amd/sharded_index.py b/tensor-truth_amd/sharded_index.py
--- a/tensor-truth_amd/sharded_index.py
+++ b/tensor-truth_amd/sharded_index.py
@@ -148,12 +148,13 @@
         shadow = None
         if self.fp8_shadow and 0 < q16.shape[0] <= _scan.ScanShadow.MAX_QUERIES and rows.shape[0] >= _scan.ScanShadow.MIN_ROWS:
             key = rows.data_ptr()
-            shadow = self._shadows.get(key)
-            if shadow is None:
+            entry = self._shadows.get(key)
+            if entry is None or entry[0] is not rows:
                 with self._shadow_lock:
-                    shadow = self._shadows.get(key)
-                    if shadow is None:
-                        shadow = self._shadows[key] = _scan.ScanShadow(rows)
+                    entry = self._shadows.get(key)
+                    if entry is None or entry[0] is not rows:
+                        entry = self._shadows[key] = (rows, _scan.build_shadow(rows, what="a shard"))
+            shadow = entry[1]
         return _scan.scan_topk(rows, q16, k, idx_base=base, shadow=shadow)
 
     def _local_topk(self, q16: torch.Tensor, k: int):
diff --git a/tensor-truth_amd/vector_index.py b/tensor-truth_amd/vector_index.py
--- a/tensor-truth_amd/vector_index.py
+++ b/tensor-truth_amd/vector_index.py
@@ -56,6 +56,7 @@
         self._written: Optional[torch.cuda.Event] = None
         self.fp8_shadow = os.environ.get("TT_SCAN_SHADOW", "1") != "0"
         self._shadow = None
+        self._shadow_failed = None
         self._cols: Dict[str, _mf.CodeColumn] = {}
         self._generation = 0
 
@@ -71,6 +72,7 @@
             grown = torch.empty((cap, self.dim), dtype=torch.bfloat16, device=self.device)
             grown[: self.n] = self._mat[: self.n]
             self._mat = grown
+            self._shadow = None
             for col in self._cols.values():
                 col.reserve(cap)
 
@@ -174,6 +176,7 @@
                 (0, self.dim), dtype=torch.bfloat16, device=self.device)
             self._cols = {key: _mf.CodeColumn.from_device(key, self.device, col.dev[: self.n].index_select(0, idx))
                           for key, col in self._cols.items()}
+            self._shadow = None
             self._generation += 1
             self._mark_written()
             self.leaf_ids = [self.leaf_ids[i] for i in keep]
@@ -230,11 +233,23 @@
             sh = self._shadow
             if self._written is not None and (sh is None or sh.rows < self.n):
                 torch.cuda.current_stream(self.device).wait_event(self._written)
-            if sh is None or sh.base_ptr != self._mat.data_ptr() or sh.cap_rows < self.n:
-                sh = self._shadow = _scan.ScanShadow(self._mat[: self.n], cap_rows=self._mat.shape[0])
-                sh.base_ptr = self._mat.data_ptr()
-            elif sh.rows < self.n:
-                sh.extend(self._mat, self.n)
+            if self._shadow_failed is self._mat:
+                return None
+            try:
+                if sh is None or sh.matrix is not self._mat or sh.cap_rows < self.n:
+                    sh = self._shadow = None
+                    sh = _scan.build_shadow(self._mat[: self.n], cap_rows=self._mat.shape[0], what="the index matrix")
+                    if sh is None:
+                        self._shadow_failed = self._mat
+                        return None
+                    sh.matrix = self._mat
+                    self._shadow = sh
+                elif sh.rows < self.n:
+                    sh.extend(self._mat, self.n)
+            except (RuntimeError, MemoryError) as exc:
+                logger.warning("fp8 shadow not extended, bf16 scan instead: %s", exc)
+                self._shadow, self._shadow_failed = None, self._mat
+                return None
             return sh if sh.rows >= mat.shape[0] else None
 
     def search(self, query_emb: torch.Tensor, k: int, snapshot=None, filters=None):
@@ -618,6 +633,7 @@
             for ix, lo in zip(self.indexes, offs):
                 mat[lo:lo + ix.n] = ix._mat[: ix.n]
                 ix._mat = mat[lo:lo + ix.n]
+                ix._shadow = None
                 ix._mark_written()
             self._mat, self.offsets, self._stamp = mat, offs, stamp
             self._leaf_ids = [ix.leaf_ids for ix in self.indexes]
@@ -637,8 +653,8 @@
             if self.fp8_shadow and 0 < q.shape[0] <= S.MAX_QUERIES and big:
                 for m in big:
                     if m not in self._seg_shadows:
-                        self._seg_shadows[m] = S(mat[offs[m]:offs[m + 1]])
-                shadows = dict(self._seg_shadows)
+                        self._seg_shadows[m] = _scan.build_shadow(mat[offs[m]:offs[m + 1]], what=f"module {m}")
+                shadows = {m: sh for m, sh in self._seg_shadows.items() if sh is not None}
         return mat, offs, ids, shadows
 
     @staticmethod
```

Result: no change. 115.1, median of 6 (+0.4%).
